# AlexGr5/StereoVision

Hardware: AMD Instinct MI355X
Metric: disparity frames/sec + HBM GB/s, 1920x1080 D=128 win=9, 1/2/4/8 GPU (higher is better)
Workload: dtype u8

## Files before the change

stereovision_amd/csrc/sv_capi.cpp:

```cpp
#include "sv_ctx.h"

namespace {
thread_local std::string g_err;
}

namespace svc {

int fail(int code, const std::string& msg) {
    g_err = msg;
    return code;
}

int hipfail(int e, const char* what) {
    return fail(SV_EHIP, std::string(what) + ": " + hipGetErrorString((hipError_t)e));
}

const std::string& last_error_msg() { return g_err; }

int check_image(const void* a, int H, int W) {
    if (!a || H <= 0 || W <= 0) return fail(SV_EINVAL, "null image or non-positive size");
    return 0;
}

int check_match(int H, int W, int min_disp, int num_disp, int win, int cost, sv::MatchPlan* plan) {
    if (H <= 0 || W <= 0) return fail(SV_EINVAL, "non-positive image size");
    if (num_disp <= 0 || num_disp > 512) return fail(SV_EINVAL, "num_disp must be in [1, 512]");
    if (win < 1 || win > 15 || (win & 1) == 0) return fail(SV_EINVAL, "win must be odd in [1, 15]");
    if (min_disp < -2047 || min_disp + num_disp - 1 > 2047)
        return fail(SV_EINVAL, "disparity range beyond the int16 x16 map: min_disp >= -2047 and "
                               "min_disp + num_disp - 1 <= 2047 required");
    if (cost == SV_COST_SGBM) return 0;
    int rc = sv::plan_match(num_disp, win, cost, plan);
    if (rc == -34) return fail(SV_ERANGE, "cost range too large for the argmin key");
    if (rc != 0) return fail(SV_EINVAL, "unsupported (num_disp, win, cost)");
    return 0;
}

SgbmParams sgbm_reference_params(int win) {
    return {8 * 3 * win * win, 32 * 3 * win * win, 1, 63, 10, 100, 32};
}

int enqueue_speckles(sv_ctx* c, int16_t* d_img, int H, int W, int pitch, int new_val, int max_speckle_size,
                     int max_diff, hipStream_t s, int nf, long long fimg) {
    if (max_speckle_size <= 0) return 0;
    c->scratch_written(d_img);
    const size_t n = (size_t)H * W * (nf < 1 ? 1 : nf);
    SV_HIP(c->cc_parent.ensure(n * 4));
    SV_HIP(c->cc_size.ensure(n * 4));
    SV_LAUNCH(c, SV_K_SPECKLE, s,
              sv::launch_speckles(d_img, H, W, pitch, new_val, max_speckle_size, max_diff, c->cc_parent.as<int>(),
                                  c->cc_size.as<int>(), s, nf < 1 ? 1 : nf, fimg));
    return 0;
}

constexpr int kSgbmChunk = 32;
size_t sgbm_budget(int device) {
    static const long long env_gb = [] {
        const char* e = std::getenv("SV_SGBM_BUDGET_GB");
        return e ? std::atoll(e) : 0LL;
    }();
    if (env_gb > 0) return (size_t)env_gb << 30;
    size_t fr = 0, tot = 0;
    (void)device;
    if (hipMemGetInfo(&fr, &tot) != hipSuccess || fr == 0) return (size_t)8 << 30;
    return std::min<size_t>(fr / 4, (size_t)48 << 30);
}

int enqueue_sgbm(sv_ctx* c, const uint8_t* L, const uint8_t* R, int H, int W, int pitch, int min_disp,
                 int num_disp, int win, SgbmParams p, int16_t* out, int opitch, hipStream_t s, int nf,
                 long long fs_in, long long fs_out) {
    if (nf < 1) nf = 1;
    c->scratch_written(out);
    if (sv::sgbm_dp(num_disp) < 0) return fail(SV_EINVAL, "num_disp must be in [1, 512]");
    if (W > 16384) return fail(SV_EINVAL, "SGBM: width beyond 16384");
    if (p.P1 < 0 || p.P2 < 0) return fail(SV_EINVAL, "negative P1/P2");
    if (p.P2 <= p.P1) p.P2 = p.P1 + 1;
    if (p.P2 >= 349525) return fail(SV_ERANGE, "SGBM: P2 too large for the 32-bit argmin key");
    p.cap = (p.cap > 15 ? p.cap : 15) | 1;
    if (p.cap > 127) return fail(SV_EINVAL, "preFilterCap must be <= 127");
    sv::SgbmArgs a{};
    a.L = L;
    a.R = R;
    a.H = H;
    a.W = W;
    a.pitch = pitch;
    a.minD = min_disp;
    a.D = num_disp;
    a.r = win / 2;
    const int maxd = min_disp + num_disp;
    a.X0 = maxd > 0 ? maxd : 0;
    int X1 = W + (min_disp < 0 ? min_disp : 0);
    if (X1 > W) X1 = W;
    a.Wb = X1 > a.X0 ? X1 - a.X0 : 0;
    a.cap = p.cap;
    a.P1 = p.P1;
    a.P2 = p.P2;
    a.uniq = p.uniq < 0 ? 10 : p.uniq;
    a.disp12 = p.disp12;
    const long long cmax = (long long)(2 * p.cap + 63) * win * win;
    if (cmax > 65535) return fail(SV_EINVAL, "SGBM: window cost beyond 16 bits (lower preFilterCap/blockSize)");
    a.l32 = (cmax > 32767 || p.P2 > 32768) ? 1 : 0;
    a.Dp = sv::sgbm_dp(num_disp);
    const size_t vol = (size_t)H * a.Wb * a.Dp;
    const size_t lsz = a.l32 ? 4 : 2;
    const bool cost1 = sv::sgbm_cost_fused(num_disp, a.r);
    const size_t rec_frame = cost1 ? (size_t)2 * H * W * 16 : 0;
    const size_t per_frame = vol * (4 + lsz * 3) + (size_t)H * a.Wb * 8 + rec_frame;
    const size_t held = c->sg_hsum.cap + c->sg_c.cap + c->sg_l.cap + c->sg_lt.cap + c->sg_band.cap + c->sg_rec.cap;
    const size_t kSgbmBudget = std::max(sgbm_budget(c->device) + held, per_frame);
    int chunk = (int)std::max<size_t>(1, std::min<size_t>({(size_t)nf, (size_t)kSgbmChunk,
                                                            kSgbmBudget / std::max<size_t>(per_frame, 1)}));
    const bool fused = sv::sgbm_fused(chunk, num_disp);
    if (fused)
        chunk = (int)std::max<size_t>(1, std::min<size_t>({(size_t)nf, (size_t)kSgbmChunk,
                                                            kSgbmBudget / (per_frame - vol * lsz)}));
    a.fused = fused ? 1 : 0;
    SV_HIP(c->sg_hsum.ensure(vol * 2 * chunk + 256));
    SV_HIP(c->sg_c.ensure(vol * 2 * chunk + 256));
    const int nl = (a.l32 ? 1 : 0) + (fused ? 0 : 1);
    SV_HIP(c->sg_l.ensure(vol * lsz * nl * chunk + 256));
    SV_HIP(c->sg_lt.ensure(vol * (a.l32 ? 4 : 2) * chunk + 256));
    if (!c->sg_aux) {
        SV_HIP(hipStreamCreateWithFlags(&c->sg_aux, hipStreamNonBlocking));
        SV_HIP(hipEventCreateWithFlags(&c->sg_ev[0], hipEventDisableTiming));
        SV_HIP(hipEventCreateWithFlags(&c->sg_ev[1], hipEventDisableTiming));
    }
    const size_t band_bytes = (size_t)H * a.Wb * 8 * chunk;
    SV_HIP(c->sg_band.ensure(band_bytes + 256 + 64 * 128));
    a.hsum = c->sg_hsum.as<uint16_t>();
    a.C = c->sg_c.as<uint16_t>();
    a.Llr = a.l32 ? c->sg_l.p : c->sg_hsum.p;
    a.Lrl = fused ? nullptr : a.l32 ? (void*)(c->sg_l.as<int32_t>() + vol * chunk) : c->sg_l.p;
    a.Ltb = c->sg_lt.p;
    a.band = c->sg_band.p;
    a.recs = nullptr;
    if (cost1) {
        SV_HIP(c->sg_rec.ensure(rec_frame * chunk + 256));
        a.recs = c->sg_rec.as<uint4>();
    }
    a.dummy = c->sg_band.as<uint8_t>() + (band_bytes + 255) / 256 * 256;
    a.opitch = opitch;
    a.fs_in = fs_in;
    a.fs_out = fs_out;
    for (int z0 = 0; z0 < nf; z0 += chunk) {
        const int n = std::min(chunk, nf - z0);
        a.L = L + z0 * fs_in;
        a.R = R + z0 * fs_in;
        a.out = out + z0 * fs_out;
        SV_LAUNCH(c, SV_K_SGBM, s, sv::launch_sgbm(a, n, s, c->sg_aux, c->sg_ev[0], c->sg_ev[1]));
        const int rc = enqueue_speckles(c, a.out, H, W, opitch, (min_disp - 1) * 16, p.speckle_win,
                                        16 * p.speckle_range, s, n, fs_out);
        if (rc) return rc;
    }
    return 0;
}

int enqueue_disparity(sv_ctx* c, const uint8_t* L, const uint8_t* R, int H, int W, int pitch,
                      int min_disp, int num_disp, int win, int cost, int row0, int row1,
                      int16_t* out, int opitch, hipStream_t s, int nf, long long fs_in,
                      long long fs_out, bool track_margins) {
    sv::MatchPlan plan;
    int rc = check_match(H, W, min_disp, num_disp, win, cost, &plan);
    if (rc) return rc;
    if (row0 < 0) row0 = 0;
    if (row1 > H) row1 = H;
    if (row1 <= row0) return 0;
    const sv_ctx::MarginKey had = c->d16_margins;
    c->scratch_written(out);
    if (cost == SV_COST_SGBM) {
        if (row0 != 0 || row1 != H) return fail(SV_EINVAL, "SGBM cannot compute a row band (use frames)");
        return enqueue_sgbm(c, L, R, H, W, pitch, min_disp, num_disp, win, sgbm_reference_params(win), out, opitch,
                            s, nf, fs_in, fs_out);
    }
    sv::MatchParams a{};
    a.L = L;
    a.R = R;
    a.H = H;
    a.W = W;
    a.pitch = pitch;
    a.minD = min_disp;
    a.D = num_disp;
    a.win = win;
    a.r = cost == SV_COST_HOG ? 0 : win / 2;
    int maxd = min_disp + num_disp;
    a.X0 = maxd > 0 ? maxd : 0;
    a.X1 = W + (min_disp < 0 ? min_disp : 0);
    if (a.X1 > W) a.X1 = W;
    if (a.X1 < a.X0) a.X1 = a.X0;
    a.row0 = row0;
    a.row1 = row1;
    a.lpg = plan.lpg;
    a.lpg_log2 = plan.lpg == 16 ? 4 : plan.lpg == 32 ? 5 : 6;
    a.dbits = plan.dbits;
    a.pad_key = (uint32_t)((sv::max_cost(win, cost) + 1) << plan.dbits);
    a.out = out;
    a.opitch = opitch;
    a.nf = nf < 1 ? 1 : nf;
    a.fs_in = fs_in;
    a.fs_out = fs_out;
    a.fs_hist = 0;
    if (cost == SV_COST_HOG && a.X1 > a.X0) {
        const long long fh = (long long)H * W * 10;
        const size_t hb = (size_t)fh * sizeof(uint16_t) * a.nf;
        SV_HIP(c->hog[0].ensure(hb));
        SV_HIP(c->hog[1].ensure(hb));
        SV_LAUNCH(c, SV_K_HOG, s,
                  sv::launch_hog_hist_pairs(L, R, H, W, pitch, win, row0, row1, c->hog[0].as<uint16_t>(),
                                            c->hog[1].as<uint16_t>(), a.nf, a.nf > 1 ? fs_in : 0, fh, s));
        a.HL = c->hog[0].as<uint16_t>();
        a.HR = c->hog[1].as<uint16_t>();
        a.fs_hist = a.nf > 1 ? fh : 0;
    }
    if (sv::ring_split(cost, win, num_disp) && a.X1 > a.X0) {
        const long long ke = sv::ring_split_elems(a.nf, fs_out, row1, opitch);
        SV_HIP(c->keys.ensure((size_t)(2 * ke) * sizeof(uint32_t)));
        a.keys = c->keys.as<uint32_t>();
        a.keys_stride = ke;
    }
    sv_ctx::MarginKey key;
    if (track_margins && out == c->d16.as<int16_t>() && row0 == 0 && row1 == H) {
        key.valid = true;
        key.p = c->d16.p;
        key.gen = c->d16.gen;
        key.H = H;
        key.W = W;
        key.opitch = opitch;
        key.X0 = a.X0;
        key.X1 = a.X1;
        key.min_disp = min_disp;
        key.nf = a.nf;
        key.fs_out = fs_out;
        a.margins_done = had.covers(key) ? 1 : 0;
        if (a.margins_done) key = had;
    }
    SV_LAUNCH(c, SV_K_MATCH, s, sv::launch_match(a, plan, cost, s));
    if (key.valid) c->d16_margins = key;
    return 0;
}

int attach_lut(sv_ctx* c, sv::PostParams& pp, hipStream_t s, bool whole) {
    pp.lut_n = 0;
    pp.lut_shift = 0;
    pp.lut_cap = 0;
    if (pp.mode == SV_POST_NONE || pp.num_disp <= 0 || pp.num_disp > 512) return 0;
    sv_ctx::LutKey k;
    k.mode = pp.mode;
    k.min_disp = pp.min_disp;
    k.num_disp = pp.num_disp;
    k.m0 = (pp.min_disp - 1) * 16;
    k.n = whole ? pp.num_disp + 1 : (pp.num_disp + 1) * 16;
    k.minf = pp.minf;
    k.maxf = pp.maxf;
    k.rangef = pp.rangef;
    k.mdg = pp.min_disp_global;
    DevBuf& buf = whole ? c->lutw : c->lut;
    sv_ctx::LutKey& key = whole ? c->lutw_key : c->lut_key;
    hipEvent_t& ev = whole ? c->lutw_ev : c->lut_ev;
    hipStream_t& bs = whole ? c->lutw_stream : c->lut_stream;
    const size_t n = (size_t)k.n;
    float* la = buf.as<float>();
    if (!(k == key) || !ev) {
        SV_HIP(buf.ensure(whole ? (n + sv::kLutWholeSpan) * 2 * sizeof(float) : n * (2 * sizeof(float) + 1)));
        la = buf.as<float>();
        if (!ev) SV_HIP(hipEventCreateWithFlags(&ev, hipEventDisableTiming));
        int e = sv::launch_post_lut(pp, k.m0, k.n, whole ? 16 : 1, la, reinterpret_cast<uint8_t*>(la + 2 * n), la + n,
                                    s);
        if (e) return hipfail(e, "launch_post_lut");
        SV_HIP(hipEventRecord(ev, s));
        key = k;
        bs = s;
    } else if (s != bs) {
        SV_HIP(hipStreamWaitEvent(s, ev, 0));
    }
    pp.lut_a = la;
    pp.lut_b = la + n;
    pp.lut_u8 = reinterpret_cast<const uint8_t*>(la + 2 * n);
    pp.lut_m0 = k.m0;
    pp.lut_n = k.n;
    pp.lut_shift = whole ? 4 : 0;
    pp.lut_cap = whole ? k.n + sv::kLutWholeSpan : k.n;
    return 0;
}

int attach_cmap(sv_ctx* c, sv::PostParams& pp, const uint8_t* table, uint8_t* d_bgr, hipStream_t s) {
    pp.out_bgr = nullptr;
    pp.cmap = nullptr;
    if (!d_bgr) return 0;
    if (!table) return fail(SV_EINVAL, "colormap output without a table");
    SV_HIP(c->cmap.ensure(256 * sizeof(uint32_t)));
    if (!c->cmap_valid || std::memcmp(c->cmap_host, table, 768) != 0) {
        uint32_t packed[256];
        for (int i = 0; i < 256; ++i)
            packed[i] = (uint32_t)table[3 * i] | ((uint32_t)table[3 * i + 1] << 8) | ((uint32_t)table[3 * i + 2] << 16);
        SV_HIP(hipMemcpyAsync(c->cmap.p, packed, sizeof(packed), hipMemcpyHostToDevice, s));
        SV_HIP(hipStreamSynchronize(s));
        std::memcpy(c->cmap_host, table, 768);
        c->cmap_valid = true;
    }
    pp.out_bgr = d_bgr;
    pp.cmap = c->cmap.as<uint32_t>();
    return 0;
}

sv::PostParams make_post(int mode, float minf, float maxf, float rangef, float mdg, int min_disp,
                         int num_disp, float* a, uint8_t* u8, float* b) {
    sv::PostParams pp{};
    pp.mode = mode;
    pp.minf = minf;
    pp.maxf = maxf;
    pp.rangef = rangef;
    pp.min_disp_global = mdg;
    pp.min_disp = min_disp;
    pp.num_disp = num_disp;
    pp.out_a = a;
    pp.out_u8 = u8;
    pp.out_b = b;
    return pp;
}

int map_out_post(sv_ctx* c, const sv_map_out* out, int min_disp, int num_disp, int cost, bool allow_harris,
                 hipStream_t s, sv::PostParams* pp, float** disp) {
    if (!out) return fail(SV_EINVAL, "null outputs");
    const int mode = out->mode;
    if (mode != SV_POST_NONE && mode != SV_POST_DEPTH && mode != SV_POST_SCALED) return fail(SV_EINVAL, "bad post mode");
    if (mode == SV_POST_DEPTH && (!out->out_a || !out->out_u8)) return fail(SV_EINVAL, "depth post outputs missing");
    if (mode == SV_POST_SCALED && (!out->out_a || !out->out_u8 || !out->out_b || num_disp <= 0))
        return fail(SV_EINVAL, "scaled post outputs missing");
    if (mode == SV_POST_NONE && (out->out_a || out->out_u8 || out->out_b))
        return fail(SV_EINVAL, "post outputs without a post mode");
    if (out->bgr && (mode == SV_POST_NONE || !out->cmap_bgr))
        return fail(SV_EINVAL, "a colormap output needs a post mode and a table");
    if (out->harris && !allow_harris) return fail(SV_EINVAL, "the Harris output belongs to sv_depth_map_batch_dev");
    if (out->d8 && (cost == SV_COST_SGBM || num_disp < 1 || num_disp > 255))
        return fail(SV_EINVAL, "u8 disparity indices need an integer-disparity cost and num_disp <= 255");
    if (!out->disparity && !out->med16 && !out->d8 && mode == SV_POST_NONE && !out->harris)
        return fail(SV_EINVAL, "no outputs");
    *pp = make_post(mode, out->min_depth, out->max_depth, out->depth_range, out->min_disp_global, min_disp, num_disp,
                    out->out_a, out->out_u8, out->out_b);
    int rc = attach_lut(c, *pp, s, cost != SV_COST_SGBM);
    if (!rc) rc = attach_cmap(c, *pp, out->cmap_bgr, out->bgr, s);
    if (rc) return rc;
    pp->out_m16 = out->med16;
    pp->out_d8 = out->d8;
    pp->d8_base = min_disp - 1;
    *disp = out->disparity;
    return 0;
}

int check_map(int fmt, const void* map, int cost, int num_disp) {
    if (fmt != SV_MAP_M16 && fmt != SV_MAP_D8) return fail(SV_EINVAL, "map format must be SV_MAP_M16 or SV_MAP_D8");
    if (!map) return fail(SV_EINVAL, "null map");
    if (fmt == SV_MAP_D8 && (cost == SV_COST_SGBM || num_disp < 1 || num_disp > 255))
        return fail(SV_EINVAL, "u8 disparity indices need an integer-disparity cost and num_disp <= 255");
    return 0;
}

sv::PostParams map_post(int fmt, void* dst, int d8_base) {
    sv::PostParams pp = make_post(SV_POST_NONE, 0.f, 0.f, 0.f, 0.f, 0, 0, nullptr, nullptr, nullptr);
    if (fmt == SV_MAP_D8) {
        pp.out_d8 = static_cast<uint8_t*>(dst);
        pp.d8_base = d8_base;
    } else {
        pp.out_m16 = static_cast<int16_t*>(dst);
    }
    return pp;
}


int stage_pair(sv_ctx* c, const uint8_t* left, const uint8_t* right, int H, int W, int channels,
               int stride) {
    if (check_image(left, H, W) || check_image(right, H, W)) return SV_EINVAL;
    if (channels != 1 && channels != 3) return fail(SV_EINVAL, "channels must be 1 or 3");
    const size_t row = (size_t)W * channels;
    if (stride < (int)row) return fail(SV_EINVAL, "stride smaller than a row");
    const size_t n = row * H;
    SV_HIP(c->hin.ensure(2 * n));
    SV_HIP(c->gray[0].ensure((size_t)H * W));
    SV_HIP(c->gray[1].ensure((size_t)H * W));
    const uint8_t* src[2] = {left, right};
    for (int k = 0; k < 2; ++k) {
        uint8_t* dst = c->hin.as<uint8_t>() + k * n;
        if ((size_t)stride == row) {
            std::memcpy(dst, src[k], n);
        } else {
            for (int y = 0; y < H; ++y) std::memcpy(dst + y * row, src[k] + (size_t)y * stride, row);
        }
    }
    if (channels == 1) {
        SV_HIP(hipMemcpyAsync(c->gray[0].p, c->hin.p, n, hipMemcpyHostToDevice, c->stream));
        SV_HIP(hipMemcpyAsync(c->gray[1].p, c->hin.as<uint8_t>() + n, n, hipMemcpyHostToDevice, c->stream));
    } else {
        SV_HIP(c->img[0].ensure(n));
        SV_HIP(c->img[1].ensure(n));
        for (int k = 0; k < 2; ++k) {
            SV_HIP(hipMemcpyAsync(c->img[k].p, c->hin.as<uint8_t>() + k * n, n, hipMemcpyHostToDevice, c->stream));
            SV_LAUNCH(c, SV_K_GRAY, c->stream,
                      sv::launch_gray(c->img[k].as<uint8_t>(), H, W, (int)row, c->gray[k].as<uint8_t>(), c->stream));
        }
    }
    return 0;
}

int collect(sv_ctx* c, const Out* outs, int n) {
    size_t total = 0;
    for (int i = 0; i < n; ++i)
        if (outs[i].host) total += (outs[i].bytes + 255) & ~(size_t)255;
    SV_HIP(c->hout.ensure(total ? total : 256));
    size_t off = 0;
    for (int i = 0; i < n; ++i) {
        if (!outs[i].host) continue;
        SV_HIP(hipMemcpyAsync(c->hout.as<uint8_t>() + off, outs[i].dev, outs[i].bytes, hipMemcpyDeviceToHost, c->stream));
        off += (outs[i].bytes + 255) & ~(size_t)255;
    }
    SV_HIP(hipStreamSynchronize(c->stream));
    off = 0;
    for (int i = 0; i < n; ++i) {
        if (!outs[i].host) continue;
        std::memcpy(outs[i].host, c->hout.as<uint8_t>() + off, outs[i].bytes);
        off += (outs[i].bytes + 255) & ~(size_t)255;
    }
    return 0;
}

int make_undistort(const double* K, const double* dist, int ndist, const double* R, const double* P,
                   int p_cols, int H, int W, sv::UndistortParams* out) {
    if (!K || H <= 0 || W <= 0) return fail(SV_EINVAL, "bad map arguments");
    if (H > 32767 || W > 32767) return fail(SV_EINVAL, "map size beyond the int16 coordinate range");
    if (!(ndist == 0 || ndist == 4 || ndist == 5 || ndist == 8 || ndist == 12 || ndist == 14) ||
        (ndist > 0 && !dist))
        return fail(SV_EINVAL, "distCoeffs must have 0, 4, 5, 8, 12 or 14 elements");
    if (ndist == 14 && (dist[12] != 0.0 || dist[13] != 0.0))
        return fail(SV_EINVAL, "tilted sensor model (tauX, tauY != 0) is not supported");
    if (P && p_cols != 3 && p_cols != 4) return fail(SV_EINVAL, "P must be 3x3 or 3x4");
    double A[9], Rm[9] = {1, 0, 0, 0, 1, 0, 0, 0, 1}, M[9];
    for (int i = 0; i < 3; ++i)
        for (int j = 0; j < 3; ++j) A[i * 3 + j] = P ? P[i * p_cols + j] : K[i * 3 + j];
    if (R) std::memcpy(Rm, R, sizeof(Rm));
    for (int i = 0; i < 3; ++i)
        for (int j = 0; j < 3; ++j)
            M[i * 3 + j] = (A[i * 3 + 0] * Rm[0 * 3 + j] + A[i * 3 + 1] * Rm[1 * 3 + j]) + A[i * 3 + 2] * Rm[2 * 3 + j];
    auto a = [&](int i, int j) { return M[i * 3 + j]; };
    const double det = a(0, 0) * (a(1, 1) * a(2, 2) - a(2, 1) * a(1, 2)) -
                       a(0, 1) * (a(1, 0) * a(2, 2) - a(2, 0) * a(1, 2)) +
                       a(0, 2) * (a(1, 0) * a(2, 1) - a(2, 0) * a(1, 1));
    if (det == 0.0) return fail(SV_EINVAL, "singular newCameraMatrix * R");
    const double d = 1.0 / det;
    double* b = out->ir;
    b[0] = (a(1, 1) * a(2, 2) - a(1, 2) * a(2, 1)) * d;
    b[1] = (a(0, 2) * a(2, 1) - a(0, 1) * a(2, 2)) * d;
    b[2] = (a(0, 1) * a(1, 2) - a(0, 2) * a(1, 1)) * d;
    b[3] = (a(1, 2) * a(2, 0) - a(1, 0) * a(2, 2)) * d;
    b[4] = (a(0, 0) * a(2, 2) - a(0, 2) * a(2, 0)) * d;
    b[5] = (a(0, 2) * a(1, 0) - a(0, 0) * a(1, 2)) * d;
    b[6] = (a(1, 0) * a(2, 1) - a(1, 1) * a(2, 0)) * d;
    b[7] = (a(0, 1) * a(2, 0) - a(0, 0) * a(2, 1)) * d;
    b[8] = (a(0, 0) * a(1, 1) - a(0, 1) * a(1, 0)) * d;
    out->fx = K[0];
    out->fy = K[4];
    out->u0 = K[2];
    out->v0 = K[5];
    for (int i = 0; i < 12; ++i) out->k[i] = i < ndist ? dist[i] : 0.0;
    out->H = H;
    out->W = W;
    return 0;
}

int check_remap(const void* src, int sH, int sW, int channels, int pitch, const void* map1, int H, int W,
                const void* dst) {
    if (!src || !map1 || !dst || sH <= 0 || sW <= 0 || H <= 0 || W <= 0)
        return fail(SV_EINVAL, "bad remap arguments");
    if (channels != 1 && channels != 3) return fail(SV_EINVAL, "channels must be 1 or 3");
    if (pitch < sW * channels) return fail(SV_EINVAL, "source pitch smaller than a row");
    return 0;
}

}

int sv::set_error(int code, const std::string& msg) { return fail(code, msg); }

extern "C" {

int sv_version(void) { return SV_API_VERSION; }

const char* sv_last_error(void) { return g_err.c_str(); }

int sv_device_count(int* n) {
    if (!n) return fail(SV_EINVAL, "null output");
    int k = 0;
    hipError_t e = hipGetDeviceCount(&k);
    if (e != hipSuccess) {
        *n = 0;
        return hipfail((int)e, "hipGetDeviceCount");
    }
    *n = k;
    return 0;
}

int sv_create(int device, sv_ctx** out) {
    if (!out) return fail(SV_EINVAL, "null output");
    *out = nullptr;
    int n = 0;
    if (hipGetDeviceCount(&n) != hipSuccess || n <= 0) return fail(SV_ENODEV, "no HIP device visible");
    if (device < 0 || device >= n) return fail(SV_ENODEV, "device index out of range");
    sv_ctx* c = new (std::nothrow) sv_ctx();
    if (!c) return fail(SV_ENOMEM, "context allocation failed");
    c->device = device;
    hipError_t e = hipSetDevice(device);
    if (e == hipSuccess) e = hipStreamCreateWithFlags(&c->stream, hipStreamNonBlocking);
    if (e != hipSuccess) {
        delete c;
        return hipfail((int)e, "sv_create");
    }
    *out = c;
    return 0;
}

void sv_destroy(sv_ctx* c) {
    if (!c) return;
    {
        std::lock_guard<std::mutex> lk(c->mu);
        (void)hipSetDevice(c->device);
        (void)hipStreamSynchronize(c->stream);
        c->prof_drain();
        for (auto e : c->pool) (void)hipEventDestroy(e);
        DevBuf* bufs[] = {&c->img[0], &c->img[1], &c->gray[0], &c->gray[1], &c->d16, &c->fa, &c->fb,
                          &c->fc, &c->u8, &c->harris, &c->hog[0], &c->hog[1], &c->fin, &c->lut,
                          &c->rmap1, &c->rmap2, &c->rdst[0], &c->rdst[1], &c->stats, &c->sel,
                          &c->sg_hsum, &c->sg_c, &c->sg_l, &c->sg_lt, &c->sg_band, &c->cc_parent,
                          &c->hist_copies, &c->cmap, &c->bgr, &c->m16,
                          &c->cc_size, &c->sg_rec, &c->gm16, &c->keys, &c->lutw, &c->fuse, &c->flow};
        if (c->lut_ev) (void)hipEventDestroy(c->lut_ev);
        if (c->lutw_ev) (void)hipEventDestroy(c->lutw_ev);
        if (c->scr_ev) (void)hipEventDestroy(c->scr_ev);
        if (c->xev) (void)hipEventDestroy(c->xev);
        if (c->sev) (void)hipEventDestroy(c->sev);
        if (c->gev) (void)hipEventDestroy(c->gev);
        for (auto e : c->wev)
            if (e) (void)hipEventDestroy(e);
        if (c->region_open) {
            (void)hipEventDestroy(c->region.a);
            (void)hipEventDestroy(c->region.b);
        }
        for (auto e : c->dev_done)
            if (e) (void)hipEventDestroy(e);
        for (auto e : c->tmr)
            if (e) (void)hipEventDestroy(e);
        if (c->sg_aux) {
            (void)hipStreamSynchronize(c->sg_aux);
            (void)hipStreamDestroy(c->sg_aux);
        }
        for (auto e : c->sg_ev)
            if (e) (void)hipEventDestroy(e);
        for (auto* b : bufs) b->release();
        c->hin.release();
        c->hout.release();
        (void)hipStreamDestroy(c->stream);
    }
    delete c;
}

int sv_event_record(sv_ctx* c, int slot, void* stream) {
    SV_ENTER(c);
    if (slot < 0 || slot >= 16) return fail(SV_EINVAL, "event slot must be in [0, 16)");
    hipEvent_t& e = c->wev[slot];
    if (!e) SV_HIP(hipEventCreateWithFlags(&e, hipEventDisableTiming));
    SV_HIP(hipEventRecord(e, pick(c, stream)));
    return 0;
}

int sv_stream_wait_event(sv_ctx* c, int slot, void* stream) {
    SV_ENTER(c);
    if (slot < 0 || slot >= 16 || !c->wev[slot]) return fail(SV_EINVAL, "event slot never recorded");
    SV_HIP(hipStreamWaitEvent(pick(c, stream), c->wev[slot], 0));
    return 0;
}

int sv_release_scratch(sv_ctx* c) {
    SV_ENTER(c);
    SV_HIP(hipStreamSynchronize(c->stream));
    if (c->sg_aux) SV_HIP(hipStreamSynchronize(c->sg_aux));
    DevBuf* bufs[] = {&c->img[0], &c->img[1], &c->gray[0], &c->gray[1], &c->d16, &c->fa, &c->fb, &c->fc,
                      &c->u8, &c->harris, &c->hog[0], &c->hog[1], &c->fin, &c->sg_hsum, &c->sg_c,
                      &c->sg_l, &c->sg_lt, &c->sg_band, &c->sg_rec, &c->cc_parent, &c->cc_size, &c->m16,
                      &c->gm16, &c->keys, &c->flow};
    for (auto* b : bufs) b->release();
    c->d16_margins.valid = false;
    return 0;
}

int sv_synchronize(sv_ctx* c) {
    SV_ENTER(c);
    SV_HIP(hipStreamSynchronize(c->stream));
    return 0;
}

void* sv_stream(sv_ctx* c) { return c ? static_cast<void*>(c->stream) : nullptr; }

int sv_plan(int num_disp, int win, int cost, int* dpl, int* lpg, int* lds_bytes) {
    sv::MatchPlan p;
    int rc = sv::plan_match(num_disp, win, cost, &p);
    if (rc == -34) return fail(SV_ERANGE, "cost range too large for the argmin key");
    if (rc) return fail(SV_EINVAL, "unsupported (num_disp, win, cost)");
    if (dpl) *dpl = p.dpl;
    if (lpg) *lpg = p.lpg;
    if (lds_bytes) *lds_bytes = (int)sv::match_lds_bytes(p, cost == SV_COST_HOG ? 0 : win / 2, cost);
    return 0;
}

int sv_dev_alloc(sv_ctx* c, uint64_t bytes, void** out) {
    SV_ENTER(c);
    if (!out || bytes == 0) return fail(SV_EINVAL, "bad allocation request");
    *out = nullptr;
    SV_HIP(hipMalloc(out, (size_t)bytes));
    return 0;
}

int sv_dev_free(sv_ctx* c, void* p) {
    SV_ENTER(c);
    if (p) SV_HIP(hipFree(p));
    return 0;
}

int sv_copy_to_device(sv_ctx* c, void* dst, const void* src, uint64_t bytes, void* stream) {
    SV_ENTER(c);
    if (!dst || !src) return fail(SV_EINVAL, "null pointer");
    if (!bytes) return 0;
    if (stream) {
        SV_HIP(hipMemcpyAsync(dst, src, (size_t)bytes, hipMemcpyHostToDevice, static_cast<hipStream_t>(stream)));
        return 0;
    }
    SV_HIP(hipMemcpyAsync(dst, src, (size_t)bytes, hipMemcpyHostToDevice, c->stream));
    SV_HIP(hipStreamSynchronize(c->stream));
    return 0;
}

int sv_copy_to_host(sv_ctx* c, void* dst, const void* src, uint64_t bytes, void* stream) {
    SV_ENTER(c);
    if (!dst || !src) return fail(SV_EINVAL, "null pointer");
    if (!bytes) return 0;
    if (stream) {
        SV_HIP(hipMemcpyAsync(dst, src, (size_t)bytes, hipMemcpyDeviceToHost, static_cast<hipStream_t>(stream)));
        return 0;
    }
    SV_HIP(hipStreamSynchronize(c->stream));
    SV_HIP(hipMemcpyAsync(dst, src, (size_t)bytes, hipMemcpyDeviceToHost, c->stream));
    SV_HIP(hipStreamSynchronize(c->stream));
    return 0;
}

int sv_profile_enable(sv_ctx* c, int on) {
    SV_ENTER(c);
    c->prof = on != 0;
    while (c->prof && c->pool.size() + 2 * c->pending.size() < 1024) {
        hipEvent_t e = nullptr;
        if (hipEventCreate(&e) != hipSuccess) break;
        c->pool.push_back(e);
    }
    return 0;
}

int sv_profile_read(sv_ctx* c, int kernel, double* total_ms, long long* count) {
    SV_ENTER(c);
    if (kernel < 0 || kernel >= SV_NKERNELS) return fail(SV_EINVAL, "kernel id out of range");
    c->prof_drain();
    if (total_ms) *total_ms = c->acc_ms[kernel];
    if (count) *count = c->cnt[kernel];
    return 0;
}

int sv_timer_begin(sv_ctx* c, void* stream) {
    SV_ENTER(c);
    for (auto& e : c->tmr)
        if (!e) SV_HIP(hipEventCreate(&e));
    SV_HIP(hipEventRecord(c->tmr[0], pick(c, stream)));
    return 0;
}

int sv_timer_end(sv_ctx* c, void* stream, double* ms) {
    SV_ENTER(c);
    if (!c->tmr[0] || !ms) return fail(SV_EINVAL, "sv_timer_end without sv_timer_begin");
    SV_HIP(hipEventRecord(c->tmr[1], pick(c, stream)));
    SV_HIP(hipEventSynchronize(c->tmr[1]));
    float f = 0.f;
    SV_HIP(hipEventElapsedTime(&f, c->tmr[0], c->tmr[1]));
    *ms = f;
    return 0;
}

int sv_profile_region_begin(sv_ctx* c, int kernel, void* stream) {
    SV_ENTER(c);
    if (kernel < 0 || kernel >= SV_NKERNELS) return fail(SV_EINVAL, "kernel id out of range");
    if (c->region_open) return fail(SV_EINVAL, "profiling regions do not nest");
    if (!c->prof) return 0;
    c->region.a = c->get_event();
    c->region.b = c->get_event();
    c->region.kid = kernel;
    SV_HIP(hipEventRecord(c->region.a, pick(c, stream)));
    c->region_open = true;
    return 0;
}

int sv_profile_region_end(sv_ctx* c, void* stream) {
    SV_ENTER(c);
    if (!c->region_open) return 0;
    c->region_open = false;
    SV_HIP(hipEventRecord(c->region.b, pick(c, stream)));
    c->pending.push_back(c->region);
    return 0;
}

int sv_profile_reset(sv_ctx* c) {
    SV_ENTER(c);
    c->prof_drain();
    for (int k = 0; k < SV_NKERNELS; ++k) {
        c->acc_ms[k] = 0.0;
        c->cnt[k] = 0;
    }
    return 0;
}

}
```

stereovision_amd/csrc/sv_capi_dev.cpp:

```cpp
#include "sv_ctx.h"

extern "C" {

int sv_gray_dev(sv_ctx* c, const uint8_t* d_bgr, int H, int W, int pitch, uint8_t* d_gray, void* stream) {
    SV_ENTER(c);
    if (check_image(d_bgr, H, W) || !d_gray) return fail(SV_EINVAL, "bad gray arguments");
    hipStream_t s = pick(c, stream);
    SV_LAUNCH(c, SV_K_GRAY, s, sv::launch_gray(d_bgr, H, W, pitch, d_gray, s));
    return 0;
}

int sv_disparity_dev(sv_ctx* c, const uint8_t* d_left, const uint8_t* d_right, int H, int W, int pitch,
                     int min_disp, int num_disp, int win, int cost, int row0, int row1, int16_t* d_disp16,
                     int out_pitch, void* stream) {
    SV_ENTER(c);
    if (check_image(d_left, H, W) || check_image(d_right, H, W) || !d_disp16)
        return fail(SV_EINVAL, "bad disparity arguments");
    if (pitch < W || out_pitch < W) return fail(SV_EINVAL, "pitch smaller than width");
    hipStream_t s = pick(c, stream);
    SV_SCRATCH(c, s);
    return enqueue_disparity(c, d_left, d_right, H, W, pitch, min_disp, num_disp, win, cost, row0, row1,
                             d_disp16, out_pitch, s);
}

int sv_median_rows_dev(sv_ctx* c, const int16_t* d_disp16, int H, int W, int row0, int row1, int min_disp,
                       int num_disp, int cost, const sv_map_out* out, void* stream) {
    SV_ENTER(c);
    if (check_image(d_disp16, H, W)) return fail(SV_EINVAL, "bad median arguments");
    if ((long long)H * W >= (1LL << 30)) return fail(SV_EINVAL, "frame too large for the median kernel");
    if (row0 < 0) row0 = 0;
    if (row1 > H) row1 = H;
    hipStream_t s = pick(c, stream);
    SV_SCRATCH(c, s);
    sv::PostParams pp;
    float* disp = nullptr;
    int rc = map_out_post(c, out, min_disp, num_disp, cost, false, s, &pp, &disp);
    if (rc) return rc;
    SV_LAUNCH(c, SV_K_MEDIAN, s, sv::launch_median_i16(d_disp16, H, W, row0, row1, disp, pp, s));
    return 0;
}

int sv_post_m16_dev(sv_ctx* c, const int16_t* d_med16, int64_t n, int mode, float min_depth, float max_depth,
                    float depth_range, float min_disp_global, int min_disp, int num_disp, float* d_disparity,
                    float* d_out_a, uint8_t* d_out_u8, float* d_out_b, void* stream) {
    SV_ENTER(c);
    if (n < 0 || (n > 0 && !d_med16)) return fail(SV_EINVAL, "bad median map");
    if (mode != SV_POST_NONE && mode != SV_POST_DEPTH && mode != SV_POST_SCALED) return fail(SV_EINVAL, "bad mode");
    if (mode == SV_POST_NONE && !d_disparity) return fail(SV_EINVAL, "no outputs");
    if (mode == SV_POST_DEPTH && (!d_out_a || !d_out_u8)) return fail(SV_EINVAL, "depth post outputs missing");
    if (mode == SV_POST_SCALED && (!d_out_a || !d_out_u8 || !d_out_b || num_disp <= 0))
        return fail(SV_EINVAL, "scaled post outputs missing");
    if (n == 0) return 0;
    hipStream_t s = pick(c, stream);
    SV_SCRATCH(c, s);
    sv::PostParams pp = make_post(mode, min_depth, max_depth, depth_range, min_disp_global, min_disp, num_disp,
                                  d_out_a, d_out_u8, d_out_b);
    int rc = attach_lut(c, pp, s);
    if (rc) return rc;
    SV_LAUNCH(c, SV_K_POST, s, sv::launch_post_m16(d_med16, (long long)n, d_disparity, pp, s));
    return 0;
}

int sv_disparity_batch_dev(sv_ctx* c, const uint8_t* d_left, const uint8_t* d_right, int n_frames, int H,
                           int W, int pitch, int64_t frame_stride, int min_disp, int num_disp, int win,
                           int cost, int16_t* d_disp16, int out_pitch, int64_t out_frame_stride,
                           void* stream) {
    SV_ENTER(c);
    if (check_image(d_left, H, W) || check_image(d_right, H, W) || !d_disp16 || n_frames < 0)
        return fail(SV_EINVAL, "bad disparity arguments");
    if (pitch < W || out_pitch < W) return fail(SV_EINVAL, "pitch smaller than width");
    if (n_frames > 1 && (frame_stride < (int64_t)pitch * H || out_frame_stride < (int64_t)out_pitch * H))
        return fail(SV_EINVAL, "frame stride smaller than a frame");
    if (n_frames == 0) return 0;
    hipStream_t s = pick(c, stream);
    SV_SCRATCH(c, s);
    return enqueue_disparity(c, d_left, d_right, H, W, pitch, min_disp, num_disp, win, cost, 0, H, d_disp16,
                             out_pitch, s, n_frames, frame_stride, out_frame_stride);
}

int sv_depth_map_batch_dev(sv_ctx* c, const uint8_t* d_left, const uint8_t* d_right, int n_frames, int H, int W,
                           int pitch, int64_t frame_stride, int min_disp, int num_disp, int win, int cost, int stages,
                           int16_t* d_disp16, const sv_map_out* out, void* stream) {
    SV_ENTER(c);
    if (stages != SV_STAGE_ALL && stages != SV_STAGE_MATCH && stages != SV_STAGE_MEDIAN)
        return fail(SV_EINVAL, "stages must be SV_STAGE_MATCH, SV_STAGE_MEDIAN or SV_STAGE_ALL");
    const bool match = stages & SV_STAGE_MATCH, median = stages & SV_STAGE_MEDIAN;
    if (n_frames < 0 || H <= 0 || W <= 0) return fail(SV_EINVAL, "bad depth-map arguments");
    if (match && (check_image(d_left, H, W) || check_image(d_right, H, W)))
        return fail(SV_EINVAL, "bad depth-map arguments");
    if (!d_disp16 && stages != SV_STAGE_ALL)
        return fail(SV_EINVAL, "the stages run apart exchange the int16 maps through d_disp16");
    if (median && !out) return fail(SV_EINVAL, "null outputs");
    if (median && out->harris && check_image(d_left, H, W)) return fail(SV_EINVAL, "Harris needs the left frames");
    if (pitch < W) return fail(SV_EINVAL, "pitch smaller than width");
    if (n_frames > 1 && frame_stride < (int64_t)pitch * H) return fail(SV_EINVAL, "frame stride smaller than a frame");
    if ((long long)H * W >= (1LL << 30)) return fail(SV_EINVAL, "frame too large for the median kernel");
    if (n_frames == 0) return 0;
    hipStream_t s = pick(c, stream);
    SV_SCRATCH(c, s);
    const long long fs = (long long)H * W;
    int16_t* d16 = d_disp16;
    if (!d16) {
        SV_HIP(c->d16.ensure((size_t)n_frames * fs * sizeof(int16_t)));
        d16 = c->d16.as<int16_t>();
    }
    if (match) {
        const int rc = enqueue_disparity(c, d_left, d_right, H, W, pitch, min_disp, num_disp, win, cost, 0, H, d16, W,
                                         s, n_frames, frame_stride, fs, !d_disp16);
        if (rc) return rc;
    }
    if (!median) return 0;
    sv::PostParams pp;
    float* disp = nullptr;
    int rc = map_out_post(c, out, min_disp, num_disp, cost, true, s, &pp, &disp);
    if (rc) return rc;
    pp.lut_unchecked = match && cost != SV_COST_SGBM && pp.lut_shift == 4 && pp.lut_m0 == (min_disp - 1) * 16 &&
                       pp.lut_n == num_disp + 1;
    const long long fin = n_frames > 1 ? frame_stride : 0;
    if (out->harris && (W < 8 || H < 8)) {
        SV_LAUNCH(c, SV_K_MEDIAN, s, sv::launch_median_i16(d16, H, W, 0, H, disp, pp, s, n_frames, fs, fs));
        SV_LAUNCH(c, SV_K_HARRIS, s, sv::launch_harris(d_left, H, W, pitch, out->harris, s, n_frames, fin, fs));
        return 0;
    }
    sv::HarrisParams hp{d_left, pitch, fin, out->harris, fs, 0, 0};
    SV_LAUNCH(c, SV_K_MEDIAN, s,
              sv::launch_median_i16(d16, H, W, 0, H, disp, pp, s, n_frames, fs, fs, out->harris ? &hp : nullptr));
    return 0;
}

int sv_harris_dev(sv_ctx* c, const uint8_t* d_gray, int H, int W, int pitch, float* d_out, void* stream) {
    SV_ENTER(c);
    if (check_image(d_gray, H, W) || !d_out) return fail(SV_EINVAL, "bad harris arguments");
    hipStream_t s = pick(c, stream);
    SV_LAUNCH(c, SV_K_HARRIS, s, sv::launch_harris(d_gray, H, W, pitch, d_out, s));
    return 0;
}

int sv_harris_batch_dev(sv_ctx* c, const uint8_t* d_gray, int n_frames, int H, int W, int pitch,
                        int64_t frame_stride, float* d_out, void* stream) {
    SV_ENTER(c);
    if (check_image(d_gray, H, W) || !d_out || n_frames < 0) return fail(SV_EINVAL, "bad harris arguments");
    if (pitch < W) return fail(SV_EINVAL, "pitch smaller than width");
    if (n_frames > 1 && frame_stride < (int64_t)pitch * H) return fail(SV_EINVAL, "frame stride smaller than a frame");
    if (n_frames == 0) return 0;
    hipStream_t s = pick(c, stream);
    SV_LAUNCH(c, SV_K_HARRIS, s,
              sv::launch_harris(d_gray, H, W, pitch, d_out, s, n_frames, (long long)frame_stride,
                                (long long)H * W));
    return 0;
}

int sv_hog_hist_dev(sv_ctx* c, const uint8_t* d_gray, int H, int W, int pitch, int win, int row0, int row1,
                    uint16_t* d_out, void* stream) {
    SV_ENTER(c);
    if (check_image(d_gray, H, W) || !d_out) return fail(SV_EINVAL, "bad hog arguments");
    if (win < 1 || win > 15 || (win & 1) == 0) return fail(SV_EINVAL, "win must be odd in [1, 15]");
    hipStream_t s = pick(c, stream);
    SV_LAUNCH(c, SV_K_HOG, s, sv::launch_hog_hist(d_gray, H, W, pitch, win, row0, row1, d_out, s));
    return 0;
}

int sv_gray(sv_ctx* c, const uint8_t* bgr, int H, int W, int stride, uint8_t* gray) {
    SV_ENTER(c);
    SV_SCRATCH(c, c->stream);
    if (check_image(bgr, H, W) || !gray) return fail(SV_EINVAL, "bad gray arguments");
    const size_t row = (size_t)W * 3, n = row * H;
    if (stride < (int)row) return fail(SV_EINVAL, "stride smaller than a row");
    SV_HIP(c->hin.ensure(n));
    for (int y = 0; y < H; ++y) std::memcpy(c->hin.as<uint8_t>() + y * row, bgr + (size_t)y * stride, row);
    SV_HIP(c->img[0].ensure(n));
    SV_HIP(c->gray[0].ensure((size_t)H * W));
    SV_HIP(hipMemcpyAsync(c->img[0].p, c->hin.p, n, hipMemcpyHostToDevice, c->stream));
    SV_LAUNCH(c, SV_K_GRAY, c->stream,
              sv::launch_gray(c->img[0].as<uint8_t>(), H, W, (int)row, c->gray[0].as<uint8_t>(), c->stream));
    Out o[] = {{gray, c->gray[0].p, (size_t)H * W}};
    return collect(c, o, 1);
}

int sv_disparity(sv_ctx* c, const uint8_t* left, const uint8_t* right, int H, int W, int channels, int stride,
                 int min_disp, int num_disp, int win, int cost, int16_t* disp16, float* harris) {
    SV_ENTER(c);
    SV_SCRATCH(c, c->stream);
    if (!disp16) return fail(SV_EINVAL, "null disparity output");
    sv::MatchPlan plan;
    int rc = check_match(H, W, min_disp, num_disp, win, cost, &plan);
    if (rc) return rc;
    rc = stage_pair(c, left, right, H, W, channels, stride);
    if (rc) return rc;
    SV_HIP(c->d16.ensure((size_t)H * W * sizeof(int16_t)));
    rc = enqueue_disparity(c, c->gray[0].as<uint8_t>(), c->gray[1].as<uint8_t>(), H, W, W, min_disp, num_disp,
                           win, cost, 0, H, c->d16.as<int16_t>(), W, c->stream);
    if (rc) return rc;
    if (harris) {
        SV_HIP(c->harris.ensure((size_t)H * W * sizeof(float)));
        SV_LAUNCH(c, SV_K_HARRIS, c->stream,
                  sv::launch_harris(c->gray[0].as<uint8_t>(), H, W, W, c->harris.as<float>(), c->stream));
    }
    Out o[] = {{disp16, c->d16.p, (size_t)H * W * sizeof(int16_t)},
               {harris, c->harris.p, (size_t)H * W * sizeof(float)}};
    return collect(c, o, 2);
}

int sv_disparity_rows(sv_ctx* c, const uint8_t* left, const uint8_t* right, int H, int W, int channels,
                      int stride, int min_disp, int num_disp, int win, int cost, int row0, int row1,
                      int16_t* disp16) {
    SV_ENTER(c);
    SV_SCRATCH(c, c->stream);
    if (!disp16) return fail(SV_EINVAL, "null disparity output");
    if (row0 < 0) row0 = 0;
    if (row1 > H) row1 = H;
    if (row1 <= row0) return 0;
    sv::MatchPlan plan;
    int rc = check_match(H, W, min_disp, num_disp, win, cost, &plan);
    if (rc) return rc;
    rc = stage_pair(c, left, right, H, W, channels, stride);
    if (rc) return rc;
    SV_HIP(c->d16.ensure((size_t)H * W * sizeof(int16_t)));
    rc = enqueue_disparity(c, c->gray[0].as<uint8_t>(), c->gray[1].as<uint8_t>(), H, W, W, min_disp, num_disp,
                           win, cost, row0, row1, c->d16.as<int16_t>(), W, c->stream);
    if (rc) return rc;
    const size_t off = (size_t)row0 * W;
    Out o[] = {{disp16 + off, c->d16.as<int16_t>() + off, (size_t)(row1 - row0) * W * sizeof(int16_t)}};
    return collect(c, o, 1);
}


int sv_median5_f32(sv_ctx* c, const float* in, int H, int W, float* out) {
    SV_ENTER(c);
    SV_SCRATCH(c, c->stream);
    if (check_image(in, H, W) || !out) return fail(SV_EINVAL, "bad median arguments");
    const size_t n = (size_t)H * W * sizeof(float);
    SV_HIP(c->hin.ensure(n));
    SV_HIP(c->fin.ensure(n));
    SV_HIP(c->fa.ensure(n));
    std::memcpy(c->hin.p, in, n);
    SV_HIP(hipMemcpyAsync(c->fin.p, c->hin.p, n, hipMemcpyHostToDevice, c->stream));
    SV_LAUNCH(c, SV_K_MEDIAN, c->stream, sv::launch_median_f32(c->fin.as<float>(), H, W, c->fa.as<float>(), c->stream));
    Out o[] = {{out, c->fa.p, n}};
    return collect(c, o, 1);
}

static int post_common(sv_ctx* c, const float* disparity, int n, const sv::PostParams& tmpl, float* a,
                       uint8_t* u8, float* b) {
    if (!disparity || n <= 0) return fail(SV_EINVAL, "bad post arguments");
    const size_t nb = (size_t)n * sizeof(float);
    SV_HIP(c->hin.ensure(nb));
    SV_HIP(c->fin.ensure(nb));
    SV_HIP(c->fa.ensure(nb));
    SV_HIP(c->fb.ensure(nb));
    SV_HIP(c->u8.ensure((size_t)n));
    std::memcpy(c->hin.p, disparity, nb);
    SV_HIP(hipMemcpyAsync(c->fin.p, c->hin.p, nb, hipMemcpyHostToDevice, c->stream));
    sv::PostParams pp = tmpl;
    pp.out_a = c->fa.as<float>();
    pp.out_u8 = c->u8.as<uint8_t>();
    pp.out_b = c->fb.as<float>();
    SV_LAUNCH(c, SV_K_POST, c->stream, sv::launch_post(c->fin.as<float>(), n, pp, c->stream));
    Out o[] = {{a, c->fa.p, nb}, {u8, c->u8.p, (size_t)n}, {b, c->fb.p, nb}};
    return collect(c, o, 3);
}

int sv_depth_post(sv_ctx* c, const float* disparity, int n, float min_depth, float max_depth, float depth_range,
                  float min_disp_global, float* depth_final, uint8_t* depth_normalized) {
    SV_ENTER(c);
    SV_SCRATCH(c, c->stream);
    if (!depth_final || !depth_normalized) return fail(SV_EINVAL, "null outputs");
    sv::PostParams pp = make_post(SV_POST_DEPTH, min_depth, max_depth, depth_range, min_disp_global, 0, 0,
                                  nullptr, nullptr, nullptr);
    return post_common(c, disparity, n, pp, depth_final, depth_normalized, nullptr);
}

int sv_scaled_post(sv_ctx* c, const float* disparity, int n, int min_disp, int num_disp,
                   float* disparity_normalized, uint8_t* normalized_u8, float* confidence) {
    SV_ENTER(c);
    SV_SCRATCH(c, c->stream);
    if (!disparity_normalized || !normalized_u8 || !confidence || num_disp <= 0)
        return fail(SV_EINVAL, "bad scaled post arguments");
    sv::PostParams pp = make_post(SV_POST_SCALED, 0.f, 0.f, 0.f, 0.f, min_disp, num_disp, nullptr, nullptr,
                                  nullptr);
    return post_common(c, disparity, n, pp, disparity_normalized, normalized_u8, confidence);
}

}

namespace {

std::mutex g_reg_mu;
std::map<uintptr_t, size_t> g_reg;

bool host_registered(const void* p, size_t bytes) {
    if (!p) return false;
    const uintptr_t a = reinterpret_cast<uintptr_t>(p);
    std::lock_guard<std::mutex> lk(g_reg_mu);
    auto it = g_reg.upper_bound(a);
    if (it == g_reg.begin()) return false;
    --it;
    return a >= it->first && a + bytes <= it->first + it->second;
}

int stage_rows(sv_ctx* c, const uint8_t* src, int y0, int y1, size_t row, int stride, uint8_t* stage, uint8_t* dev,
               int nsub) {
    if ((size_t)stride == row) {
        SV_HIP(hipMemcpyAsync(dev + (size_t)y0 * row, src + (size_t)y0 * row, (size_t)(y1 - y0) * row,
                              hipMemcpyHostToDevice, c->stream));
        return 0;
    }
    sv::HostPool& pool = sv::HostPool::get();
    for (int k = 0; k < nsub; ++k) {
        const int a0 = y0 + (int)((long long)(y1 - y0) * k / nsub), a1 = y0 + (int)((long long)(y1 - y0) * (k + 1) / nsub);
        if (a1 <= a0) continue;
        const int parts = pool.threads();
        pool.parallel_for(parts, [&](int p) {
            const int a = a0 + (int)((long long)(a1 - a0) * p / parts), b = a0 + (int)((long long)(a1 - a0) * (p + 1) / parts);
            if (b <= a) return;
            if ((size_t)stride == row)
                std::memcpy(stage + (size_t)a * row, src + (size_t)a * row, (size_t)(b - a) * row);
            else
                for (int y = a; y < b; ++y) std::memcpy(stage + (size_t)y * row, src + (size_t)y * stride, row);
        });
        SV_HIP(hipMemcpyAsync(dev + (size_t)a0 * row, stage + (size_t)a0 * row, (size_t)(a1 - a0) * row,
                              hipMemcpyHostToDevice, c->stream));
    }
    return 0;
}

int host_lut(sv_ctx* c, const sv::PostParams& pp) {
    if (c->hl_valid && c->hl_key == c->lut_key) return 0;
    const size_t n = (size_t)pp.lut_n;
    try {
        c->hl_a.resize(n);
        c->hl_b.resize(n);
        c->hl_u8.resize(n);
    } catch (...) {
        return fail(SV_ENOMEM, "host table allocation failed");
    }
    SV_HIP(hipMemcpyAsync(c->hl_a.data(), pp.lut_a, n * sizeof(float), hipMemcpyDeviceToHost, c->stream));
    SV_HIP(hipMemcpyAsync(c->hl_b.data(), pp.lut_b, n * sizeof(float), hipMemcpyDeviceToHost, c->stream));
    SV_HIP(hipMemcpyAsync(c->hl_u8.data(), pp.lut_u8, n, hipMemcpyDeviceToHost, c->stream));
    SV_HIP(hipStreamSynchronize(c->stream));
    c->hl_key = c->lut_key;
    c->hl_valid = true;
    return 0;
}

struct FrameOut {
    float* a;
    float* disp;
    uint8_t* u8;
    float* b;
    uint8_t* bgr;
};

template <bool U8, bool SCALED, bool BGR>
int expand_rows(const int16_t* med, size_t a, size_t b, int m0, int nl, const HostEnt* ent, const float* lb,
                const FrameOut& o) {
    for (size_t i = a; i < b; ++i) o.disp[i] = (float)med[i] * 0.0625f;
    int nbad = 0;
    for (size_t i = a; i < b; ++i) {
        const uint32_t li = (uint32_t)(med[i] - m0);
        if (__builtin_expect(li >= (uint32_t)nl, 0)) {
            ++nbad;
            continue;
        }
        const HostEnt e = ent[li];
        o.a[i] = e.a;
        if (U8) o.u8[i] = (uint8_t)e.ubgr;
        if (SCALED) o.b[i] = lb[li];
        if (BGR) {
            const uint32_t v = e.ubgr >> 8;
            uint8_t* d = o.bgr + 3 * i;
            if (i + 1 < b) std::memcpy(d, &v, 4);
            else std::memcpy(d, &v, 3);
        }
    }
    return nbad;
}

struct HostProf {
    std::atomic<bool> on{std::getenv("SV_HOST_PROFILE") != nullptr};
    bool print = std::getenv("SV_HOST_PROFILE") != nullptr;
    std::mutex mu;
    double t[6] = {0, 0, 0, 0, 0, 0};
    double acc[6] = {0, 0, 0, 0, 0, 0};
    long n = 0, nacc = 0;
    void add(const double* d) {
        std::lock_guard<std::mutex> lk(mu);
        for (int i = 0; i < 6; ++i) {
            t[i] += d[i];
            acc[i] += d[i];
        }
        ++nacc;
        if (print && ++n % 200 == 0) {
            std::fprintf(stderr, "[sv host] per call (ms): prepare %.3f  stage+issue %.3f  wait-first %.3f  expand %.3f  "
                         "wait-rest %.3f  total %.3f\n", t[0] / n, t[1] / n, t[2] / n, t[3] / n, t[4] / n, t[5] / n);
            for (double& v : t) v = 0;
            n = 0;
        }
    }
};
HostProf& host_prof() {
    static HostProf* p = new HostProf();
    return *p;
}
int env_int(const char* name, int dflt, int lo, int hi) {
    const char* e = std::getenv(name);
    if (!e) return dflt;
    const int v = std::atoi(e);
    return v < lo ? lo : v > hi ? hi : v;
}
double now_ms() {
    return std::chrono::duration<double, std::milli>(std::chrono::steady_clock::now().time_since_epoch()).count();
}

int host_frame_path(sv_ctx* c, const uint8_t* left, const uint8_t* right, int H, int W, int channels, int stride,
                    int min_disp, int num_disp, int win, int cost, sv::PostParams pp, const uint8_t* table,
                    FrameOut o) {
    const bool prof = host_prof().on;
    double tm[6] = {0, 0, 0, 0, 0, 0}, t0 = prof ? now_ms() : 0, tp = t0;
    sv::MatchPlan plan;
    int rc = check_match(H, W, min_disp, num_disp, win, cost, &plan);
    if (rc) return rc;
    if ((long long)H * W >= (1LL << 30)) return fail(SV_EINVAL, "frame too large");
    if (check_image(left, H, W) || check_image(right, H, W)) return SV_EINVAL;
    if (channels != 1 && channels != 3) return fail(SV_EINVAL, "channels must be 1 or 3");
    const size_t row = (size_t)W * channels;
    if (stride < (int)row) return fail(SV_EINVAL, "stride smaller than a row");
    const size_t n = (size_t)H * W;
    SV_HIP(c->hin.ensure(2 * row * H));
    SV_HIP(c->gray[0].ensure(n));
// ... 1036 lines not shown
```

stereovision_amd/csrc/sv_ctx.h:

```cpp
#pragma once
#include <cstdio>
#include <cstdlib>
#include <algorithm>
#include <chrono>
#include <cstring>
#include <map>
#include <mutex>
#include <thread>
#include <new>
#include <string>
#include <vector>

#include "sv_internal.h"
#include "sv_pool.h"
#include "../../include/stereovision_amd.h"

namespace svc {
int fail(int code, const std::string& msg);
int hipfail(int e, const char* what);
const std::string& last_error_msg();
}
using svc::fail;
using svc::hipfail;

#define SV_HIP(call)                                               \
    do {                                                           \
        hipError_t e_ = (call);                                    \
        if (e_ != hipSuccess) return hipfail((int)e_, #call);      \
    } while (0)

#define SV_LAUNCH(ctx, kid, stream, call)                          \
    do {                                                           \
        (ctx)->prof_begin((kid), (stream));                        \
        int e_ = (call);                                           \
        if (e_ != 0) {                                             \
            (ctx)->prof_abort();                                   \
            return hipfail(e_, #call);                             \
        }                                                          \
        (ctx)->prof_end((stream));                                 \
    } while (0)

struct DevBuf {
    void* p = nullptr;
    size_t cap = 0;
    unsigned long long gen = 0;
    hipError_t ensure(size_t n) {
        if (n <= cap) return hipSuccess;
        ++gen;
        if (p) (void)hipFree(p);
        p = nullptr;
        cap = 0;
        hipError_t e = hipMalloc(&p, n);
        if (e == hipSuccess) cap = n;
        return e;
    }
    void release() {
        ++gen;
        if (p) (void)hipFree(p);
        p = nullptr;
        cap = 0;
    }
    hipError_t ensure_zeroed(size_t n) {
        if (n <= cap) return hipSuccess;
        hipError_t e = ensure(n);
        if (e == hipSuccess) e = hipMemset(p, 0, cap);
        if (e == hipSuccess) e = hipDeviceSynchronize();
        return e;
    }
    template <class T> T* as() const { return static_cast<T*>(p); }
};

struct HostBuf {
    void* p = nullptr;
    size_t cap = 0;
    hipError_t ensure(size_t n) {
        if (n <= cap) return hipSuccess;
        if (p) (void)hipHostFree(p);
        p = nullptr;
        cap = 0;
        hipError_t e = hipHostMalloc(&p, n, hipHostMallocDefault);
        if (e == hipSuccess) cap = n;
        return e;
    }
    void release() {
        if (p) (void)hipHostFree(p);
        p = nullptr;
        cap = 0;
    }
    template <class T> T* as() const { return static_cast<T*>(p); }
};

struct EvPair {
    hipEvent_t a, b;
    int kid;
};

struct HostEnt {
    float a;
    uint32_t ubgr;
};

struct sv_ctx {
    int device = 0;
    hipStream_t stream = nullptr;
    std::mutex mu;
    DevBuf img[2], gray[2], d16, fa, fb, fc, u8, harris, hog[2], fin, lut, rmap1, rmap2, rdst[2], stats, sel,
        sg_hsum, sg_c, sg_l, sg_lt, sg_band, sg_rec, cc_parent, cc_size, hist_copies, cmap, bgr;
    DevBuf fuse;
    DevBuf flow;
    uint8_t cmap_host[768] = {};
    bool cmap_valid = false;
    DevBuf m16;
    DevBuf gm16;
    DevBuf keys;
    std::vector<float> hl_a, hl_b;
    std::vector<uint8_t> hl_u8;
    std::vector<HostEnt> hl_ent;
    bool hl_valid = false;
    hipEvent_t dev_done[8] = {};
    hipEvent_t tmr[2] = {nullptr, nullptr};
    hipStream_t sg_aux = nullptr;
    hipEvent_t sg_ev[2] = {nullptr, nullptr};
    struct LutKey {
        int mode = -1, min_disp = 0, num_disp = 0, m0 = 0, n = 0;
        float minf = 0, maxf = 0, rangef = 0, mdg = 0;
        bool operator==(const LutKey& o) const {
            return mode == o.mode && min_disp == o.min_disp && num_disp == o.num_disp && m0 == o.m0 &&
                   n == o.n && std::memcmp(&minf, &o.minf, sizeof(float)) == 0 &&
                   std::memcmp(&maxf, &o.maxf, sizeof(float)) == 0 &&
                   std::memcmp(&rangef, &o.rangef, sizeof(float)) == 0 &&
                   std::memcmp(&mdg, &o.mdg, sizeof(float)) == 0;
        }
    } lut_key, hl_key;
    hipEvent_t lut_ev = nullptr;
    hipStream_t lut_stream = nullptr;
    DevBuf lutw;
    LutKey lutw_key;
    hipEvent_t lutw_ev = nullptr;
    hipStream_t lutw_stream = nullptr;
    HostBuf hin, hout;
    struct MarginKey {
        bool valid = false;
        const void* p = nullptr;
        unsigned long long gen = 0;
        int H = 0, W = 0, opitch = 0, X0 = 0, X1 = 0, min_disp = 0, nf = 0;
        long long fs_out = 0;
        bool covers(const MarginKey& o) const {
            return valid && p == o.p && gen == o.gen && H == o.H && W == o.W && opitch == o.opitch &&
                   X0 == o.X0 && X1 == o.X1 && min_disp == o.min_disp && nf >= o.nf &&
                   (o.nf <= 1 || fs_out == o.fs_out);
        }
    } d16_margins;
    void scratch_written(const void* out) {
        const char* b = static_cast<const char*>(d16.p);
        const char* o = static_cast<const char*>(out);
        if (b && o >= b && o < b + d16.cap) d16_margins.valid = false;
    }
    hipStream_t scr_stream = nullptr;
    hipEvent_t scr_ev = nullptr;
    hipEvent_t xev = nullptr;
    hipEvent_t sev = nullptr;
    hipEvent_t gev = nullptr;
    hipEvent_t wev[16] = {};
    bool prof = false;
    std::vector<EvPair> pending;
    std::vector<hipEvent_t> pool;
    double acc_ms[SV_NKERNELS] = {};
    long long cnt[SV_NKERNELS] = {};
    EvPair cur{};
    bool cur_open = false;
    EvPair region{};
    bool region_open = false;

    hipEvent_t get_event() {
        if (!pool.empty()) {
            hipEvent_t e = pool.back();
            pool.pop_back();
            return e;
        }
        hipEvent_t e = nullptr;
        (void)hipEventCreate(&e);
        return e;
    }
    void prof_begin(int kid, hipStream_t s) {
        if (!prof) return;
        cur.a = get_event();
        cur.b = get_event();
        cur.kid = kid;
        cur_open = true;
        (void)hipEventRecord(cur.a, s);
    }
    void prof_end(hipStream_t s) {
        if (!prof || !cur_open) return;
        (void)hipEventRecord(cur.b, s);
        pending.push_back(cur);
        cur_open = false;
    }
    void prof_abort() {
        if (!cur_open) return;
        pool.push_back(cur.a);
        pool.push_back(cur.b);
        cur_open = false;
    }
    void prof_drain() {
        for (auto& p : pending) {
            (void)hipEventSynchronize(p.b);
            float ms = 0.f;
            if (hipEventElapsedTime(&ms, p.a, p.b) == hipSuccess) {
                acc_ms[p.kid] += ms;
                cnt[p.kid] += 1;
            }
            pool.push_back(p.a);
            pool.push_back(p.b);
        }
        pending.clear();
    }
};

inline hipStream_t pick(sv_ctx* c, void* s) { return s ? static_cast<hipStream_t>(s) : c->stream; }

struct ProfScope {
    sv_ctx* c;
    hipStream_t s;
    bool ok = false;
    ProfScope(sv_ctx* ctx, int kid, hipStream_t stream) : c(ctx), s(stream) { c->prof_begin(kid, s); }
    void done() { ok = true; }
    ~ProfScope() {
        if (ok) c->prof_end(s);
        else c->prof_abort();
    }
};

namespace svc {

struct SgbmParams {
    int P1, P2, disp12, cap, uniq, speckle_win, speckle_range;
};
SgbmParams sgbm_reference_params(int win);

int check_image(const void* a, int H, int W);
int check_match(int H, int W, int min_disp, int num_disp, int win, int cost, sv::MatchPlan* plan);
int enqueue_speckles(sv_ctx* c, int16_t* d_img, int H, int W, int pitch, int new_val, int max_speckle_size,
                     int max_diff, hipStream_t s, int nf = 1, long long fimg = 0);
int enqueue_sgbm(sv_ctx* c, const uint8_t* L, const uint8_t* R, int H, int W, int pitch, int min_disp,
                 int num_disp, int win, SgbmParams p, int16_t* out, int opitch, hipStream_t s, int nf = 1,
                 long long fs_in = 0, long long fs_out = 0);
int enqueue_disparity(sv_ctx* c, const uint8_t* L, const uint8_t* R, int H, int W, int pitch,
                      int min_disp, int num_disp, int win, int cost, int row0, int row1,
                      int16_t* out, int opitch, hipStream_t s, int nf = 1, long long fs_in = 0,
                      long long fs_out = 0, bool track_margins = false);
int attach_lut(sv_ctx* c, sv::PostParams& pp, hipStream_t s, bool whole = false);
int attach_cmap(sv_ctx* c, sv::PostParams& pp, const uint8_t* table, uint8_t* d_bgr, hipStream_t s);
sv::PostParams make_post(int mode, float minf, float maxf, float rangef, float mdg, int min_disp,
                         int num_disp, float* a, uint8_t* u8, float* b);

int map_out_post(sv_ctx* c, const sv_map_out* out, int min_disp, int num_disp, int cost, bool allow_harris,
                 hipStream_t s, sv::PostParams* pp, float** disp);

struct MapOut {
    int fmt = 0;
    void* map = nullptr;
    int d8_base = 0;
    size_t el() const { return fmt == SV_MAP_D8 ? 1 : 2; }
};
int check_map(int fmt, const void* map, int cost, int num_disp);
sv::PostParams map_post(int fmt, void* dst, int d8_base);

int stage_pair(sv_ctx* c, const uint8_t* left, const uint8_t* right, int H, int W, int channels, int stride);

struct Out {
    void* host;
    const void* dev;
    size_t bytes;
};
int collect(sv_ctx* c, const Out* outs, int n);

int make_undistort(const double* K, const double* dist, int ndist, const double* R, const double* P,
                   int p_cols, int H, int W, sv::UndistortParams* out);
int check_remap(const void* src, int sH, int sW, int channels, int pitch, const void* map1, int H, int W,
                const void* dst);

}
using namespace svc;

struct ScratchUse {
    sv_ctx* c;
    hipStream_t s;
    int rc = 0;
    ScratchUse(sv_ctx* ctx, hipStream_t stream) : c(ctx), s(stream) {
        if (c->scr_stream && c->scr_stream != s && c->scr_ev) {
            hipError_t e = hipStreamWaitEvent(s, c->scr_ev, 0);
            if (e != hipSuccess) rc = hipfail((int)e, "hipStreamWaitEvent (context scratch)");
        }
    }
    ~ScratchUse() {
        if (!c->scr_ev && hipEventCreateWithFlags(&c->scr_ev, hipEventDisableTiming) != hipSuccess) {
            c->scr_ev = nullptr;
            return;
        }
        if (hipEventRecord(c->scr_ev, s) == hipSuccess) c->scr_stream = s;
    }
};

#define SV_SCRATCH(ctx, stream)                                             \
    ScratchUse scratch_(ctx, stream);                                       \
    if (scratch_.rc) return scratch_.rc

struct Guard {
    sv_ctx* c;
    std::unique_lock<std::mutex> lk;
    int rc = 0;
    explicit Guard(sv_ctx* ctx) : c(ctx), lk(ctx->mu) {
        hipError_t e = hipSetDevice(ctx->device);
        if (e != hipSuccess) rc = hipfail((int)e, "hipSetDevice");
    }
};

#define SV_ENTER(ctx)                                                       \
    if (!(ctx)) return fail(SV_EINVAL, "null context");                     \
    Guard guard_(ctx);                                                      \
    if (guard_.rc) return guard_.rc
```

stereovision_amd/csrc/sv_internal.h:

```cpp
#pragma once
#include <hip/hip_runtime.h>
#include <stdint.h>

#include <cstdlib>
#include <string>

struct sv_comm;

namespace sv {

__device__ __forceinline__ void sad_u32_acc(uint32_t& a, uint32_t b, uint32_t c) {
    asm("v_sad_u32 %0, %0, %1, %2" : "+v"(a) : "v"(b), "v"(c));
}

__device__ __forceinline__ int clampi(int v, int lo, int hi) { return min(max(v, lo), hi); }

__device__ __forceinline__ int bgr_to_gray(int b, int g, int r) {
    return (b * 1868 + g * 9617 + r * 4899 + (1 << 13)) >> 14;
}

inline bool env_flag(const char* name, bool default_on) {
    const char* e = std::getenv(name);
    return default_on ? !(e && e[0] == '0') : (e && e[0] == '1');
}
inline int env_int(const char* name, int lo, int hi) {
    const char* e = std::getenv(name);
    const int v = e ? std::atoi(e) : 0;
    return v >= lo && v <= hi ? v : 0;
}

int set_error(int code, const std::string& msg);

int comm_group_start();
int comm_group_end();
int comm_send(sv_comm* c, const void* buf, size_t bytes, int peer, hipStream_t s);
int comm_recv(sv_comm* c, void* buf, size_t bytes, int peer, hipStream_t s);
int comm_rank(const sv_comm* c);
int comm_size(const sv_comm* c);
int comm_device(const sv_comm* c);

enum Cost { COST_SAD = 0, COST_SSD = 1, COST_HOG = 2, COST_SGBM = 3 };

struct MatchPlan {
    int dpl;
    int lpg;
    int ndw;
    int dbits;
    int mfma_only = 0;
};

struct MatchParams {
    const uint8_t* L;
    const uint8_t* R;
    const uint16_t* HL;
    const uint16_t* HR;
    int H, W, pitch;
    int minD, D, r;
    int win;
    int X0, X1;
    int row0, row1;
    int lpg, lpg_log2, dbits;
    int16_t* out;
    int opitch;
    int nf;
    long long fs_in, fs_out, fs_hist;
    uint32_t pad_key;
    int segm;
    alignas(16) int xcd_map;
    uint32_t* keys;
    long long keys_stride;
    int margins_done;
};

int plan_match(int num_disp, int win, int cost, MatchPlan* plan);
uint64_t max_cost(int win, int cost);
size_t match_lds_bytes(const MatchPlan& p, int r, int cost);
int launch_match(const MatchParams& a, const MatchPlan& p, int cost, hipStream_t s);
bool ring_split(int cost, int win, int num_disp);
bool ring_ssd(int cost, int win, int num_disp);
bool ssd_mfma(int cost, int win, int num_disp);
bool ssd_mfma_fits(const MatchParams& a, int cost);
int launch_ssd_mfma(const MatchParams& a, hipStream_t s);
long long ring_split_elems(int nf, long long fs_out, int row1, int opitch);
int launch_fill_i16(int16_t* out, int opitch, int H, int W, int16_t v, hipStream_t s);

int launch_gray(const uint8_t* bgr, int H, int W, int pitch, uint8_t* gray, hipStream_t s);
int launch_harris(const uint8_t* g, int H, int W, int pitch, float* out, hipStream_t s, int nf = 1,
                  long long fs_in = 0, long long fs_out = 0);
int launch_hog_hist(const uint8_t* g, int H, int W, int pitch, int win, int row0, int row1,
                    uint16_t* hist, hipStream_t s);
int launch_hog_hist_pairs(const uint8_t* g0, const uint8_t* g1, int H, int W, int pitch, int win, int row0,
                          int row1, uint16_t* h0, uint16_t* h1, int nf, long long fs_in, long long fs_hist,
                          hipStream_t s);

struct UndistortParams {
    double ir[9];
    double fx, fy, u0, v0;
    double k[12];
    int H, W;
};
int launch_undistort_map(const UndistortParams& p, short2* map1, uint16_t* map2, hipStream_t s);
int launch_remap(const uint8_t* src, int sH, int sW, int channels, int spitch, long long sfs,
                 const short2* map1, const uint16_t* map2, int H, int W, bool gray_out, uint8_t* dst,
                 int dpitch, long long dfs, int nf, hipStream_t s);

int launch_resize_linear(const void* src, int sH, int sW, int cn, int spitch, long long sfs, void* dst,
                         int dH, int dW, int dpitch, long long dfs, int nf, bool f32, hipStream_t s);

struct FrameStatsArgs {
    const uint8_t* img0;
    const uint8_t* img1;
    int H, W, pitch, cn;
    int bh, bw;
    uint32_t* block_sum;
    uint32_t* block_sq;
    uint32_t* hist;
    uint32_t* hist_copies;
    int per;
    long long fs;
};
constexpr int kHistCopies = 8;
int launch_frame_stats(const FrameStatsArgs& a, int nimg, hipStream_t s);

enum SelectMask { SEL_ALL = 0, SEL_POSITIVE = 1, SEL_MASK_GT = 2 };
constexpr int kMaxRanks = 4;
constexpr int kSelBatch = 16;
struct SelectArgs {
    const float* x;
    const float* mask;
    float thr;
    int mask_mode;
    size_t n;
    int shift, bits;
    int nranks;
    int narr;
    size_t xstride, mstride;
    uint32_t prefix[kSelBatch][kMaxRanks];
    uint32_t* ghist;
    unsigned long long* counts;
    uint32_t* hist_out;
    unsigned long long* counts_out;
};
constexpr int kCountSlots = 32;
int launch_select_hist(const SelectArgs& a, hipStream_t s);

enum AffineMode { AFF_F32 = 0, AFF_F64 = 1, AFF_FILL = 2 };
struct AffineArgs {
    const float* x;
    float* out;
    size_t n;
    int mode;
    float fa, fb, fc, fd;
    double ds, doff;
};
int launch_affine_f32(const AffineArgs& a, hipStream_t s);

struct GaussArgs {
    const float* src;
    float* dst;
    int H, W, r;
    float c[16];
};
enum FuseBase { FUSE_BASE_STEREO = 0, FUSE_BASE_MIDAS = 1, FUSE_BASE_FLOW = 2 };
struct FuseBlendArgs {
    const float* stereo;
    const float* conf;
    const float* midas;
    const float* flow;
    float* fused;
    uint32_t* stats;
    int H, W, base;
    int midas_fill, flow_fill;
    int r;
    float sw, mfw, thr, hthr, k1, k2;
    float c[16];
};
constexpr int kBilateralMaxR = 7;
constexpr int kBilateralMaxTaps = 148;
constexpr int kBilateralLut = 4096 + 2;
struct BilateralArgs {
    const float* src;
    const float* lut;
    float* dst_f32;
    uint8_t* dst_u8;
    uint8_t* dst_bgr;
    const uint32_t* cmap;
    uint32_t* stats;
    int H, W, r, ntaps;
    float scale;
    float sw[kBilateralMaxTaps];
    short off[kBilateralMaxTaps];
};
int bilateral_taps(int r, int* dy, int* dx);
int launch_gauss_f32(const GaussArgs& a, hipStream_t s);
int launch_fuse_blend(const FuseBlendArgs& a, hipStream_t s);
int launch_bilateral_f32(BilateralArgs a, const float* space_w, hipStream_t s);
constexpr int kFuseSlots = 32, kFuseSlotStride = 32;
constexpr size_t kFuseStatsBytes = (size_t)kFuseSlots * kFuseSlotStride * sizeof(uint32_t);
inline void fuse_stats_fold(const uint32_t* slots, uint32_t w[4]) {
    w[0] = w[1] = w[2] = w[3] = 0;
    for (int s = 0; s < kFuseSlots; ++s) {
        const uint32_t* p = slots + s * kFuseSlotStride;
        w[0] = p[0] > w[0] ? p[0] : w[0];
        w[1] = p[1] > w[1] ? p[1] : w[1];
        w[2] += p[2];
        w[3] += p[3];
    }
}
inline float fuse_stat_decode(uint32_t k) {
    const uint32_t u = (k & 0x80000000u) ? (k ^ 0x80000000u) : ~k;
    float f;
    __builtin_memcpy(&f, &u, sizeof f);
    return f;
}
inline float fuse_stat_min(const uint32_t* w) { return fuse_stat_decode(~w[0]); }
inline float fuse_stat_max(const uint32_t* w) { return fuse_stat_decode(w[1]); }

constexpr int kFbMaxPolyN = 7;
constexpr int kFbMaxWin = 31;
struct FbPolyArgs {
    const float* src;
    float* R;
    size_t plane;
    int H, W, n;
    float g[kFbMaxPolyN + 1], xg[kFbMaxPolyN + 1], xxg[kFbMaxPolyN + 1];
    double ig11, ig03, ig33, ig55;
};
struct FbUpdateArgs {
    const float* R0;
    const float* R1;
    const float* flow;
    float* M;
    size_t plane;
    int H, W;
};
struct FbSolveArgs {
    const float* M;
    size_t plane;
    float* flow;
    int interleaved;
    int H, W, m;
    double scale;
};
struct FlowDepthArgs {
    const float* flow;
    float* depth;
    float* stable;
    uint32_t* stats;
    int H, W;
    double m[9];
    float alpha, beta;
};
int launch_fb_u8_f32(const uint8_t* src, int H, int W, int pitch, float* dst, hipStream_t s);
int launch_fb_scale(float* x, size_t n, float k, hipStream_t s);
int launch_fb_polyexp(const FbPolyArgs& a, hipStream_t s);
int launch_fb_update_matrices(const FbUpdateArgs& a, hipStream_t s);
int launch_fb_blur_solve(const FbSolveArgs& a, hipStream_t s);
int launch_flow_depth(const FlowDepthArgs& a, hipStream_t s);

struct SgbmArgs {
    const uint8_t* L;
    const uint8_t* R;
    int H, W, pitch;
    int minD, D, r;
    int Dp;
    int X0, Wb;
    int cap, P1, P2, uniq, disp12;
    uint16_t* hsum;
    uint16_t* C;
    void* Llr;
    void* Lrl;
    void* Ltb;
    int l32;
    int fused;
    uint4* recs;
    void* band;
    int16_t* out;
    int opitch;
    void* dummy;
    long long fs_in, fs_out;
    __device__ __forceinline__ void select_frame(int z) {
        const size_t vol = (size_t)H * Wb * Dp * z;
        L += z * fs_in;
        R += z * fs_in;
        out += z * fs_out;
        hsum += vol;
        C += vol;
        const size_t lb = vol * (l32 ? 4 : 2);
        Llr = static_cast<char*>(Llr) + lb;
        Lrl = static_cast<char*>(Lrl) + lb;
        Ltb = static_cast<char*>(Ltb) + lb;
        band = static_cast<char*>(band) + (size_t)H * Wb * 8 * z;
        if (recs) recs += (size_t)2 * H * W * z;
    }
};
int sgbm_dp(int D);
bool sgbm_fused(int nf, int D);
bool sgbm_cost_fused(int D, int r);
int launch_sgbm(const SgbmArgs& a, int nf, hipStream_t s, hipStream_t aux, hipEvent_t fork, hipEvent_t join);
int launch_speckles(int16_t* img, int H, int W, int pitch, int newv, int maxsize, int maxdiff, int* parent,
                    int* size, hipStream_t s, int nf = 1, long long fimg = 0);

enum PostMode { POST_NONE = 0, POST_DEPTH = 1, POST_SCALED = 2 };
struct PostParams {
    int mode;
    float minf, maxf, rangef, min_disp_global;
    int min_disp, num_disp;
    float* out_a;
    uint8_t* out_u8;
    float* out_b;
    uint8_t* out_bgr;
    const uint32_t* cmap;
    int16_t* out_m16;
    uint8_t* out_d8;
    int d8_base;
    const float* lut_a;
    const uint8_t* lut_u8;
    const float* lut_b;
    int lut_m0, lut_n;
    int lut_shift;
    int lut_unchecked;
    int lut_cap;
};
constexpr int kLutWholeSpan = 4096;
struct HarrisParams {
    const uint8_t* g;
    int pitch;
    long long fs_in;
    float* out;
    long long fs_out;
    int mbx;
    int form;
};
int launch_median_i16(const int16_t* in, int H, int W, int row0, int row1, float* disp,
                      const PostParams& pp, hipStream_t s, int nf = 1, long long fs_in = 0,
                      long long fs_out = 0, const HarrisParams* harris = nullptr);
int launch_median_f32(const float* in, int H, int W, float* out, hipStream_t s);
int launch_post_m16(const int16_t* in, long long n, float* disp, const PostParams& pp, hipStream_t s);
int launch_post(const float* disp, int n, const PostParams& pp, hipStream_t s);
int launch_post_lut(const PostParams& pp, int m0, int n, int step, float* lut_a, uint8_t* lut_u8,
                    float* lut_b, hipStream_t s);

}
```

stereovision_amd/csrc/sv_match.hip:

```cpp
#include "sv_match_packs.h"

namespace sv {
namespace {

int seg_mult(int kind, int r) {
    static const int sm4 = env_int("SV_SAD4_SEG", 1, 8);
    if (kind != COST_SAD4) return 4;
    if (sm4) return sm4;
    return (2 * r - 2 + 3) / 4 <= 2 ? 4 : 2;
}
__host__ __device__ constexpr bool hi_keys(int cost, int r) { return cost == COST_SAD4 && r <= 5; }
template <int COST, int ND, int NW>
__device__ __forceinline__ void ccol(const Pk<NW>& l, const Pk<NW>& r, uint32_t* v) {
    if constexpr (COST == COST_SAD) {
        uint32_t a = 0u;
#pragma unroll
        for (int i = 0; i < ND; ++i) a = __builtin_amdgcn_sad_u8(l.w[i], r.w[i], a);
        v[0] = a;
    } else if constexpr (COST == COST_SAD4) {
        constexpr int NC = NW - 4;
        uint32_t s = 0u;
#pragma unroll
        for (int i = 0; i < NC; ++i) s = __builtin_amdgcn_sad_u8(l.w[i], r.w[i], s);
#pragma unroll
// ... 92 lines not shown
    }
    if constexpr (LPG == 64) {
#pragma unroll
        for (int i = 0; i < N; ++i)
            v[i] = min(v[i], (uint32_t)__builtin_amdgcn_update_dpp(-1, (int)v[i], 0x143, 0xC, 0xF, false));
    }
}

__device__ __forceinline__ void reduce_scatter16(uint32_t (&v)[16], int l) {
#define SV_RS_STEP(HALF, BIT, CTRL)                                                            \
    {                                                                                          \
        const bool hi = (l & (BIT)) != 0;                                                      \
        _Pragma("unroll") for (int k = 0; k < (HALF); ++k) {                                   \
            const uint32_t send = hi ? v[k] : v[k + (HALF)];                                   \
            const uint32_t keep = hi ? v[k + (HALF)] : v[k];                                   \
            v[k] = min(keep, (uint32_t)__builtin_amdgcn_update_dpp(0u, (int)send, CTRL, 0xF, 0xF, false)); \
        }                                                                                      \
    }
    SV_RS_STEP(8, 8, 0x140)
    SV_RS_STEP(4, 4, 0x141)
    SV_RS_STEP(2, 2, 0x1B)
    SV_RS_STEP(1, 1, 0xB1)
#undef SV_RS_STEP
}
template <int COST, int ND> struct Occ {
    static constexpr int W = COST == COST_SAD4 ? 2 : (COST == COST_SAD || ND <= 3) ? 3 : 2;
};

template <int COST, int ND, int DPL>
__global__ __launch_bounds__((64 * PackCfg<COST, ND>::WPB), (Occ<COST, ND>::W)) void k_match(MatchParams a) {
    constexpr int NW = PackCfg<COST, ND>::NW;
    constexpr int ROWS = PackCfg<COST, ND>::ROWS;
    extern __shared__ __attribute__((aligned(16))) uint4 smem[];
    if (blockIdx.z) {
        a.L += blockIdx.z * a.fs_in;
        a.R += blockIdx.z * a.fs_in;
        a.out += blockIdx.z * a.fs_out;
        if constexpr (COST == COST_HOG) {
            a.HL += blockIdx.z * a.fs_hist;
            a.HR += blockIdx.z * a.fs_hist;
        }
    }
    const int lane = threadIdx.x & 63;
    const int wid = PackCfg<COST, ND>::WPB == 1 ? 0 : (int)(threadIdx.x >> 6);
    const int LPG = a.lpg;
    const int S = seg_width(LPG, DPL, a.segm);
    const int WC = wave_cols(LPG, DPL, a.segm);
    const int r = a.r;
    const int W2 = 2 * r + 1;
    SV_MATCH_REGIONS(WC, LPG, DPL, r)
    using P = PackCfg<COST, ND>;
    uint4* wbase = reinterpret_cast<uint4*>(reinterpret_cast<char*>(smem) + (size_t)wid * (NL + NRphys) * P::SLOT_BYTES);
    typename P::CT* cbase = reinterpret_cast<typename P::CT*>(wbase + (size_t)(NL + NRphys) * P::QX);
    const PackOut<COST, ND> Lw{wbase, cbase};
    const PackOut<COST, ND> Rw{wbase + (size_t)NL * P::QX, cbase + NL};
    const PackPtr<COST, ND> Lp{Lw.x, Lw.c};
    const PackPtr<COST, ND> Rp{Rw.x, Rw.c};

    const int y = a.row0 + ((int)blockIdx.y * PackCfg<COST, ND>::WPB + wid) * ROWS;
    const int yc = min(y, a.row1 - 1);
    const int xw = a.X0 + (int)blockIdx.x * WC;
    const int cL0 = xw - 3 * r - 1;
    const int cR0 = cL0 - a.minD - (LPG * DPL - 1);

    build_all_packs<COST, ND, DPL>(a, yc, cL0, NL, cR0, NRlog, c0, Lw, Rw, lane);

    if (blockIdx.x == 0) {
        const int16_t inv = (int16_t)((a.minD - 1) * 16);
#pragma unroll
        for (int q = 0; q < ROWS; ++q) {
            if (y + q >= a.row1) break;
            int16_t* orow = a.out + (size_t)(y + q) * a.opitch;
            for (int x = lane; x < a.X0; x += 64) orow[x] = inv;
            for (int x = a.X1 + lane; x < a.W; x += 64) orow[x] = inv;
        }
    }
    __syncthreads();
    if (y >= a.row1) return;

    const int g = lane >> a.lpg_log2;
    const int l = lane & (LPG - 1);
    const int sl = l ^ (((lane >> 4) & 1) << 3);
    const int xs = xw + g * S;
    const int iL0 = g * S + 2 * r + 1;
    const int iR0 = g * S + 2 * r + (LPG - sl) * DPL;
    const uint32_t dmask = (1u << a.dbits) - 1u;
    const int dbits = a.dbits;
    const int j = l - (LPG - 16);

    uint32_t mk[DPL];
    uint32_t h[DPL][ROWS], bk[ROWS][DPL];
#pragma unroll
    for (int k = 0; k < DPL; ++k) {
        const int idx = sl * DPL + k;
        mk[k] = idx < a.D ? (uint32_t)idx : 0xFFFFFFFFu;
#pragma unroll
        for (int q = 0; q < ROWS; ++q) h[k][q] = idx < a.D ? (uint32_t)idx : a.pad_key | (uint32_t)idx;
    }

    for (int t = 0; t < W2; ++t) {
        const Pk<NW> L = ld<COST, ND>(Lp + (iL0 + t));
#pragma unroll
        for (int k = 0; k < DPL; ++k) {
            uint32_t vn[ROWS];
            ccol<COST, ND, NW>(L, ld<COST, ND>(Rp + rslot(iR0 + t - k, c0, DPL)), vn);
            if constexpr (COST == COST_HOG) h[k][0] = (vn[0] << dbits) | mk[k];
            else {
#pragma unroll
                for (int q = 0; q < ROWS; ++q) h[k][q] += vn[q] << dbits;
            }
        }
    }
    {
        const bool emit0 = j == 0 && xs < a.X1;
#pragma unroll
        for (int q = 0; q < ROWS; ++q) {
            uint32_t b = 0xFFFFFFFFu;
#pragma unroll
            for (int k = 0; k < DPL; ++k) b = min(b, h[k][q]);
            if (LPG == 16) reduce_batch<16, 1>(&b);
            else if (LPG == 32) reduce_batch<32, 1>(&b);
            else reduce_batch<64, 1>(&b);
            if (emit0 && y + q < a.row1)
                a.out[(size_t)(y + q) * a.opitch + xs] = key_disp16(b, dmask, a.minD);
        }
    }

    const int phi = (DPL - W2 % DPL) % DPL;
    const int cut = DPL - phi;
    const int iN = iR0 + W2;
    Pk<NW> rn[DPL], ro[DPL];
#pragma unroll
    for (int s = 1; s < DPL; ++s) {
        rn[s] = ld<COST, ND>(Rp + rslot(iN - (DPL - s), c0, DPL));
        if constexpr (COST != COST_HOG) ro[s] = ld<COST, ND>(Rp + rslot(iR0 - (DPL - s), c0, DPL));
    }
    const PackPtr<COST, ND> rn0 = Rp + rslot(iN, c0, DPL);
    const PackPtr<COST, ND> ro0 = Rp + rslot(iR0, c0, DPL);
    const PackPtr<COST, ND> ln0 = Lp + (iL0 + W2);
    const PackPtr<COST, ND> lo0 = Lp + iL0;
    const int T = (S - 1 + DPL - 1) / DPL * DPL;

    for (int t0 = 0, c = 0; t0 < T; t0 += DPL, ++c) {
        match_chunk<COST, ND, DPL>(cut, dbits, rn0 + c * (DPL + 1), ro0 + c * (DPL + 1), ln0 + t0, lo0 + t0, rn,
                                   ro, h, mk, bk);
        if constexpr (ROWS * DPL == 16 || ROWS * DPL == 32) {
            if (LPG == 16) {
#pragma unroll
                for (int half = 0; half < ROWS * DPL / 16; ++half) {
                    uint32_t v[16];
#pragma unroll
                    for (int i = 0; i < 16; ++i) v[i] = bk[(16 * half + i) / DPL][i % DPL];
                    reduce_scatter16(v, l);
                    const int q = (16 * half) / DPL + l / DPL, e = t0 + l % DPL + 1, x = xs + e;
                    if (e < S && x < a.X1 && y + q < a.row1)
                        a.out[(size_t)(y + q) * a.opitch + x] = key_disp16(v[0], dmask, a.minD);
                }
                continue;
            }
        }
        if constexpr (ROWS * DPL == 8) {
            uint32_t v[8];
#pragma unroll
            for (int i = 0; i < 8; ++i) v[i] = bk[i / DPL][i % DPL];
            reduce_scatter8_bm(v, lane & 15);
            uint32_t key = v[0];
            if (LPG >= 32) {
                const auto p = __builtin_amdgcn_permlane16_swap(key, key, false, false);
                key = min(p[0], p[1]);
            }
            if (LPG == 64) {
                const auto p = __builtin_amdgcn_permlane32_swap(key, key, false, false);
                key = min(p[0], p[1]);
            }
            const int i = (l >> 1) & 7, q = i / DPL, e = t0 + i % DPL + 1, x = xs + e;
            if (l < 16 && (l & 1) == 0 && e < S && x < a.X1 && y + q < a.row1)
                a.out[(size_t)(y + q) * a.opitch + x] = key_disp16(key, dmask, a.minD);
            continue;
        }
        const int e = t0 + j + 1;
        const int x = xs + e;
        const bool emit = j >= 0 && j < DPL && e < S && x < a.X1;
        if (LPG == 16) reduce_batch<16, ROWS * DPL>(&bk[0][0]);
        else if (LPG == 32) reduce_batch<32, ROWS * DPL>(&bk[0][0]);
        else reduce_batch<64, ROWS * DPL>(&bk[0][0]);
#pragma unroll
        for (int q = 0; q < ROWS; ++q) {
            uint32_t v = bk[q][0];
#pragma unroll
            for (int u = 1; u < DPL; ++u) v = (j == u) ? bk[q][u] : v;
            if (emit && y + q < a.row1)
                a.out[(size_t)(y + q) * a.opitch + x] = key_disp16(v, dmask, a.minD);
        }
    }
}
__global__ void k_fill_i16(int16_t* out, int opitch, int H, int W, int16_t v) {
    const int x = blockIdx.x * blockDim.x + threadIdx.x;
    const int y = blockIdx.y;
    if (x < W && y < H) out[(size_t)y * opitch + x] = v;
}

template <int COST, int ND, int DPL>
int launch_one(const MatchParams& a, size_t lds, hipStream_t s) {
    auto fn = k_match<COST, ND, DPL>;
    if (lds > 65536) {
        hipError_t e = hipFuncSetAttribute((const void*)fn, hipFuncAttributeMaxDynamicSharedMemorySize, (int)lds);
        if (e != hipSuccess) return (int)e;
    }
    const int wc = wave_cols(a.lpg, DPL, a.segm);
    const int rows_per_block = PackCfg<COST, ND>::WPB * PackCfg<COST, ND>::ROWS;
    dim3 grid((a.X1 - a.X0 + wc - 1) / wc, (a.row1 - a.row0 + rows_per_block - 1) / rows_per_block,
              a.nf > 1 ? a.nf : 1);
    hipLaunchKernelGGL(fn, grid, dim3(64 * PackCfg<COST, ND>::WPB), lds, s, a);
    return (int)hipGetLastError();
}

template <int COST, int ND>
int launch_dpl(const MatchParams& a, const MatchPlan& p, size_t lds, hipStream_t s) {
    switch (p.dpl) {
        case 4: return launch_one<COST, ND, 4>(a, lds, s);
        case 6: return launch_one<COST, ND, 6>(a, lds, s);
        case 8: return launch_one<COST, ND, 8>(a, lds, s);
    }
    return (int)hipErrorInvalidValue;
}

template <int COST>
int launch_nd(const MatchParams& a, const MatchPlan& p, size_t lds, hipStream_t s) {
    if constexpr (COST == COST_HOG) {
        return launch_dpl<COST, 5>(a, p, lds, s);
    } else if constexpr (COST == COST_SAD4) {
        switch (p.ndw) {
            case 2: return launch_dpl<COST, 2>(a, p, lds, s);
            case 3: return launch_dpl<COST, 3>(a, p, lds, s);
            case 4: return launch_dpl<COST, 4>(a, p, lds, s);
            case 5: return launch_dpl<COST, 5>(a, p, lds, s);
            case 6: return launch_dpl<COST, 6>(a, p, lds, s);
            case 7: return launch_dpl<COST, 7>(a, p, lds, s);
        }
        return (int)hipErrorInvalidValue;
    } else {
        switch (p.ndw) {
            case 1: return launch_dpl<COST, 1>(a, p, lds, s);
            case 2: return launch_dpl<COST, 2>(a, p, lds, s);
            case 3: return launch_dpl<COST, 3>(a, p, lds, s);
            case 4: return launch_dpl<COST, 4>(a, p, lds, s);
        }
        return (int)hipErrorInvalidValue;
    }
}

}

uint64_t max_cost(int win, int cost) {
    return cost == COST_SAD ? (uint64_t)win * win * 255
         : cost == COST_SSD ? (uint64_t)win * win * 255 * 255
                            : (uint64_t)9 * win * win * 255;
}

int plan_match(int num_disp, int win, int cost, MatchPlan* plan) {
    static const int menu[][2] = {{4, 16}, {6, 16}, {8, 16}, {6, 32}, {8, 32}, {6, 64}, {8, 64}};
    if (num_disp <= 0 || win < 1 || (win & 1) == 0 || win > 15) return -22;
    if (cost != COST_SAD && cost != COST_SSD && cost != COST_HOG) return -22;
    int i = 0;
    for (; i < 7; ++i)
        if (menu[i][0] * menu[i][1] >= num_disp) break;
    if (i == 7) return -22;
    plan->dpl = menu[i][0];
    plan->lpg = menu[i][1];
    const int kind = kind_of(cost, win);
    plan->ndw = kind == COST_HOG ? 5 : kind == COST_SAD4 ? win / 2
              : (win + 3) / 4;
    int n = plan->dpl * plan->lpg - 1, bits = 0;
    while (n > 0) { ++bits; n >>= 1; }
    plan->dbits = bits < 1 ? 1 : bits;
    if (hi_keys(kind, win / 2)) plan->dbits = 16;
    const uint64_t cmax = max_cost(win, cost);
    const bool over = (cmax << plan->dbits) >= (1ull << 32) ||
                      (num_disp < plan->dpl * plan->lpg && cost != COST_HOG &&
                       ((2 * cmax + 2) << plan->dbits) >= (1ull << 32));
    plan->mfma_only = 0;
    if (over) {
        if (!ssd_mfma(cost, win, num_disp)) return -34;
        plan->mfma_only = 1;
    }
    return 0;
}

size_t match_lds_bytes(const MatchPlan& p, int r, int cost) {
    const int kind = kind_of(cost, 2 * r + 1);
    const int wpb = kind == COST_SAD4 ? 1 : 4;
    SV_MATCH_REGIONS(wave_cols(p.lpg, p.dpl, seg_mult(kind, r)), p.lpg, p.dpl, r)
    return (size_t)wpb * (NL + NRphys) * pack_shape(kind, p.ndw).slot_bytes;
}

int launch_fill_i16(int16_t* out, int opitch, int H, int W, int16_t v, hipStream_t s) {
    if (H <= 0 || W <= 0) return 0;
    hipLaunchKernelGGL(k_fill_i16, dim3((W + 255) / 256, H), dim3(256), 0, s, out, opitch, H, W, v);
    return (int)hipGetLastError();
}

int launch_match(const MatchParams& a, const MatchPlan& p, int cost, hipStream_t s) {
    if (a.row1 <= a.row0) return 0;
    if (a.X1 <= a.X0) {
        for (int z = 0; z < (a.nf > 1 ? a.nf : 1); ++z) {
            int e = launch_fill_i16(a.out + z * a.fs_out + (size_t)a.row0 * a.opitch, a.opitch,
                                    a.row1 - a.row0, a.W, (int16_t)((a.minD - 1) * 16), s);
            if (e) return e;
        }
        return 0;
    }
    if (ssd_mfma_fits(a, cost)) return launch_ssd_mfma(a, s);
    if (p.mfma_only) return (int)hipErrorInvalidValue;
    const int e = launch_match_ring(a, cost, s);
    if (e >= 0) return e;
    const size_t lds = match_lds_bytes(p, a.r, cost);
    if (lds > 160 * 1024) return (int)hipErrorInvalidValue;
    MatchParams b = a;
    b.segm = seg_mult(kind_of(cost, a.win), a.r);
    switch (kind_of(cost, a.win)) {
        case COST_SAD: return launch_nd<COST_SAD>(b, p, lds, s);
        case COST_SAD4: return launch_nd<COST_SAD4>(b, p, lds, s);
        case COST_SSD: return launch_nd<COST_SSD>(b, p, lds, s);
        case COST_HOG: return launch_nd<COST_HOG>(b, p, lds, s);
    }
    return (int)hipErrorInvalidValue;
}

}
```

stereovision_amd/csrc/sv_match_ring.hip:

```cpp
#include "sv_match_packs.h"
#include "sv_xcd.h"

#include <cstdio>

namespace sv {
namespace {

typedef unsigned short u16x2 __attribute__((ext_vector_type(2)));
__device__ __forceinline__ uint32_t pk_add16(uint32_t a, uint32_t b) {
    return __builtin_bit_cast(uint32_t, __builtin_bit_cast(u16x2, a) + __builtin_bit_cast(u16x2, b));
}

typedef uint32_t lds_u32x4 __attribute__((ext_vector_type(4), may_alias));

template <int R, int LPGT, bool DEFER, bool KEYS, bool SSD = false, bool LDSMIN = false>
__global__ __launch_bounds__(64, 2) void k_match_ring(MatchParams a) {
    using P = PackCfg<COST_SAD4, R>;
    constexpr int NW = P::NW, NC = P::NC, W2 = 2 * R + 1;
    static_assert(!LDSMIN || (LPGT == 32 && R <= 5), "the LDS fold is laid out for two 32-lane groups of 32-bit keys");
    constexpr bool PK = R >= 6;
    static_assert(P::SPLIT && (P::CW == 3) == PK, "ring kind expects split packs (20 B for r 2..3, 24 B for r 4..5, 28 B for r 6..7)");
    extern __shared__ __attribute__((aligned(16))) uint4 smem[];
    int bx, by, bz;
    xcd_tile(a.xcd_map != 0, bx, by, bz);
    if (bz) {
        a.L += bz * a.fs_in;
        a.R += bz * a.fs_in;
        a.out += bz * a.fs_out;
        if constexpr (KEYS) a.keys += bz * a.fs_out;
    }
    const int lane = threadIdx.x;
    constexpr int LPG = LPGT;
    const int S = a.segm;
    constexpr int M = W2 + 1;
    constexpr int U = M % 4 == 0 ? M : M % 2 == 0 ? 2 * M : 4 * M;
    constexpr int NCH = U / 4;
    SV_RING_GEOM(LPG, S, R)
    constexpr int c0 = RING_C0;
    const int nit = (Tn + U - 1) / U;
    const int e0 = (nit * U - Tn) >> 2;
    uint4* wbase = smem + ring_scratch_bytes(LDSMIN) / 16;
    typename P::CT* cbase = reinterpret_cast<typename P::CT*>(wbase + (size_t)slots);
    const PackOut<COST_SAD4, R> Lw{wbase + RING_PAD_F, cbase + RING_PAD_F};
    const PackOut<COST_SAD4, R> Rw{wbase + NL + RING_PAD_F + RING_PAD_M, cbase + NL + RING_PAD_F + RING_PAD_M};
    const PackPtr<COST_SAD4, R> Lp{Lw.x, Lw.c};
    const PackPtr<COST_SAD4, R> Rp{Rw.x, Rw.c};

    const int y = a.row0 + by * 4;
    const int yc = min(y, a.row1 - 1);
    const int xw = a.X0 + bx * WC;
    const int cL0 = xw - R;
    const int cR0 = cL0 - a.minD - (4 * LPG - 1);
    build_ring_packs<R, 3, RG_DPL>(a, yc, cL0, NL, cR0, NRlog, c0, Lw, Rw, lane);

    if (!KEYS && bx == 0 && !a.margins_done) {
        const int16_t inv = (int16_t)((a.minD - 1) * 16);
#pragma unroll
        for (int q = 0; q < 4; ++q) {
            if (y + q >= a.row1) break;
            int16_t* orow = a.out + (size_t)(y + q) * a.opitch;
            for (int x = lane; x < a.X0; x += 64) orow[x] = inv;
            for (int x = a.X1 + lane; x < a.W; x += 64) orow[x] = inv;
        }
    }
    __syncthreads();
    if (y >= a.row1) return;

    const int g = lane / LPG;
    const int l = lane & (LPG - 1);
    const int xs = xw + g * S;
    const int dl = PK ? min(4 * l, a.D - 4) : 4 * l;
    const int iR0 = g * S + 4 * (LPG - 1) - dl + 3;
    constexpr int RQ = PK ? 2 : 4;
    uint32_t h[RG_DPL][RQ], lab[RG_DPL];
#pragma unroll
    for (int k = 0; k < RG_DPL; ++k) {
        const int idx = 4 * l + k;
        const uint32_t base = PK ? 0u : idx < a.D ? (uint32_t)idx : (SSD ? a.pad_key : 0x8000u << 16) | (uint32_t)idx;
        lab[k] = (uint32_t)idx;
#pragma unroll
        for (int q = 0; q < RQ; ++q) h[k][q] = base;
    }
    uint32_t ring[M][RG_DPL][RQ];
#pragma unroll
    for (int s = 0; s < M; ++s)
#pragma unroll
        for (int k = 0; k < RG_DPL; ++k)
#pragma unroll
            for (int q = 0; q < RQ; ++q) asm volatile("" : "=v"(ring[s][k][q]));
    Pk<NW> rn[RG_DPL];
#pragma unroll
    for (int s = 1; s < RG_DPL; ++s) rn[RG_DPL - s] = ld<COST_SAD4, R, true>(Rp + rslot(iR0 - s, c0, RG_DPL));
    PackPtr<COST_SAD4, R> rb = Rp + (rslot(iR0, c0, RG_DPL) - e0 * (RG_DPL + 1));
    PackPtr<COST_SAD4, R> lb = Lp + (g * S - 4 * e0);
    constexpr bool LPF = R != 5;
    Pk<NW> Lnext = ld<COST_SAD4, R, true>(lb + 4 * e0);
    const int jq = (lane >> 2) & 3, ju = (lane >> 1) & 1;
    constexpr bool join2 = LPG >= 32;
    int pofs = 0;
    if (join2 && !LDSMIN) {
        const auto p = __builtin_amdgcn_permlane16_swap((uint32_t)lane, (uint32_t)lane + 64u, false, false);
        pofs = (max(p[0], p[1]) < 64u) ? 0 : 2;
    }
    const int eq = LDSMIN ? lane >> 4 : jq;
    const int exs = LDSMIN ? xw + ((lane >> 2) & 1) * S : xs;
    const int eb = (LDSMIN ? ((lane >> 3) & 1) + 2 * (lane & 1) : ju + pofs) - 2 * R;
    constexpr int OB = KEYS ? 4 : 2;
    const int ooff = OB * ((y + eq) * a.opitch + exs + eb);
    const auto orsrc = KEYS ? __builtin_amdgcn_make_buffer_rsrc(a.keys, 0, 0x7FFFFFFF, 0x00020000)
                            : __builtin_amdgcn_make_buffer_rsrc(a.out, 0, 0x7FFFFFFF, 0x00020000);
    const int emax = (LDSMIN ? (lane & 2) == 0 && y + eq < a.row1
                             : (l & 1) == 0 && l < (join2 ? 32 : 16) && y + jq < a.row1)
                         ? max(0, min(S, a.X1 - exs)) : 0;

    auto emit_key = [&](uint32_t key, int tt) {
        const int off = (unsigned)(tt + eb) < (unsigned)emax ? ooff + OB * tt : (int)0x80000000u;
        if constexpr (KEYS) __builtin_amdgcn_raw_buffer_store_b32(key, orsrc, off, 0, 0);
        else __builtin_amdgcn_raw_buffer_store_b16(
            (uint16_t)key_disp16(key, SSD ? (1u << a.dbits) - 1u : 0xFFFFu, a.minD), orsrc, off, 0, 0);
    };
    auto join_pairs = [&](uint32_t kA_, uint32_t kB_) {
        auto p = __builtin_amdgcn_permlane16_swap(kA_, kB_, false, false);
        uint32_t key = min(p[0], p[1]);
        if (LPG == 64) {
            p = __builtin_amdgcn_permlane32_swap(key, key, false, false);
            key = min(p[0], p[1]);
        }
        return key;
    };
    auto join_rows = [&](uint32_t key) {
        if (LPG >= 32) {
            const auto p = __builtin_amdgcn_permlane16_swap(key, key, false, false);
            key = min(p[0], p[1]);
        }
        if (LPG == 64) {
            const auto p = __builtin_amdgcn_permlane32_swap(key, key, false, false);
            key = min(p[0], p[1]);
        }
        return key;
    };
    uint32_t dv[8], kA = 0xFFFFFFFFu;
    int tprev = -(1 << 24);
#pragma unroll
    for (int i = 0; i < 8; ++i) dv[i] = 0xFFFFFFFFu;
    [[maybe_unused]] uint32_t* const scr = reinterpret_cast<uint32_t*>(smem);
    [[maybe_unused]] const uint32_t scr_m0 = __builtin_amdgcn_readfirstlane(
        (uint32_t)(uintptr_t)(__attribute__((address_space(3))) uint32_t*)scr);
    [[maybe_unused]] const lds_u32x4* const sra = reinterpret_cast<const lds_u32x4*>(scr + 8 * lane + 4 * ((lane >> 3) & 1));
    [[maybe_unused]] const lds_u32x4* const srb = reinterpret_cast<const lds_u32x4*>(scr + 8 * lane + 4 * (1 - ((lane >> 3) & 1)));
    auto lds_fold = [&](const lds_u32x4& p, const lds_u32x4& s) {
        uint32_t m = min(min(p.x, p.y), p.z);
        m = min(min(m, p.w), s.x);
        m = min(min(m, s.y), s.z);
        m = min(m, s.w);
        m = min(m, (uint32_t)__builtin_amdgcn_update_dpp(0u, (int)m, 0xB1, 0xF, 0xF, false));
        return min(m, (uint32_t)__builtin_amdgcn_update_dpp(0u, (int)m, 0x4E, 0xF, 0xF, false));
    };
    [[maybe_unused]] const bool pairB = (lane & 1) != 0;

    constexpr int NZ = 2 * R - 4 * (2 * R / 4) + 1;
    auto chunk = [&](auto warm_c, const int ch, const int t0) __attribute__((always_inline)) {
            constexpr bool WARM = decltype(warm_c)::value;
            [[maybe_unused]] uint32_t bk[4][2];
#pragma unroll
            for (int u = 0; u < 4; ++u) {
                const int slot = (4 * ch + u) % M, oslot = (4 * ch + u + 1) % M;
                rn[u] = ld<COST_SAD4, R, true>(rb + (ch * (RG_DPL + 1) + u));
                const Pk<NW> Lc = LPF ? Lnext : ld<COST_SAD4, R, true>(lb + (4 * ch + u));
                if constexpr (LPF) Lnext = ld<COST_SAD4, R, true>(lb + (4 * ch + u + 1));
                lds_u32x4 fa{}, fb{};
                if constexpr (LDSMIN && !WARM) {
                    if ((u & 1) == 0) { fa = *sra; fb = *srb; }
                }
                uint32_t sqL[4];
                if constexpr (SSD) {
                    uint32_t sc = 0u;
#pragma unroll
                    for (int i = 0; i < NC; ++i) sc = __builtin_amdgcn_udot4(Lc.w[i], Lc.w[i], sc, false);
#pragma unroll
                    for (int q = 0; q < 4; ++q)
                        sqL[q] = __builtin_amdgcn_udot4(Lc.w[NC + q], Lc.w[NC + q], sc, false) << a.dbits;
                }
#pragma unroll
                for (int kk = 0; kk < RG_DPL; ++kk) {
                    const int k = RG_DPL - 1 - kk;
                    const Pk<NW>& Rk = rn[(u - k) & 3];
                    if constexpr (PK) {
                        uint32_t cn = 0u;
#pragma unroll
                        for (int i = 0; i < NC; ++i) cn = __builtin_amdgcn_sad_u8(Lc.w[i], Rk.w[i], cn);
                        cn |= cn << 16;
#pragma unroll
                        for (int j = 0; j < 2; ++j) {
                            const uint32_t c = __builtin_amdgcn_sad_hi_u8(
                                Lc.w[NC + 2 * j + 1], Rk.w[NC + 2 * j + 1],
                                __builtin_amdgcn_sad_u8(Lc.w[NC + 2 * j], Rk.w[NC + 2 * j], cn));
                            if constexpr (!WARM) sad_u32_acc(h[k][j], ring[oslot][k][j], c);
                            else h[k][j] = pk_add16(h[k][j], c);
                            ring[slot][k][j] = c;
                        }
                    } else if constexpr (SSD) {
                        uint32_t cn = 0u, sr = 0u;
#pragma unroll
                        for (int i = 0; i < NC; ++i) {
                            cn = __builtin_amdgcn_udot4(Lc.w[i], Rk.w[i], cn, false);
                            sr = __builtin_amdgcn_udot4(Rk.w[i], Rk.w[i], sr, false);
                        }
#pragma unroll
                        for (int q = 0; q < 4; ++q) {
                            const uint32_t lr = __builtin_amdgcn_udot4(Lc.w[NC + q], Rk.w[NC + q], cn, false);
                            const uint32_t rr = __builtin_amdgcn_udot4(Rk.w[NC + q], Rk.w[NC + q], sr, false);
                            const uint32_t t = (rr << a.dbits) + sqL[q];
                            const uint32_t c = (uint32_t)__mul24((int)lr, -(2 << a.dbits)) + t;
                            if constexpr (WARM) h[k][q] += c;
                            else sad_u32_acc(h[k][q], ring[oslot][k][q], c);
                            ring[slot][k][q] = c;
                        }
                    } else {
                        uint32_t cn = 0u;
#pragma unroll
                        for (int i = 0; i < NC; ++i) cn = __builtin_amdgcn_sad_hi_u8(Lc.w[i], Rk.w[i], cn);
#pragma unroll
                        for (int q = 0; q < 4; ++q) {
                            const uint32_t c = __builtin_amdgcn_sad_hi_u8(Lc.w[NC + q], Rk.w[NC + q], cn);
                            if constexpr (!WARM) sad_u32_acc(h[k][q], ring[oslot][k][q], c);
                            else h[k][q] += c;
                            ring[slot][k][q] = c;
                        }
                    }
                }
                if constexpr (WARM) {
                    __builtin_amdgcn_sched_barrier(0);
                    continue;
                }
#pragma unroll
                for (int q = 0; q < 4; ++q) {
                    uint32_t kq[RG_DPL];
#pragma unroll
                    for (int k = 0; k < RG_DPL; ++k)
                        kq[k] = !PK ? h[k][q] : (q & 1) ? (h[k][q >> 1] & 0xFFFF0000u) | lab[k] : (h[k][q >> 1] << 16) | lab[k];
                    bk[q][u & 1] = min(min(kq[0], kq[1]), min(kq[2], kq[3]));
                }
                if constexpr (LDSMIN) {
                    if (u == 2) {
                        kA = lds_fold(fa, fb);
                    } else if (u == 0) {
                        const uint32_t kB = lds_fold(fa, fb);
                        emit_key(pairB ? kB : kA, tprev);
                        tprev = t0;
                    }
                }
                __builtin_amdgcn_sched_barrier(0);
                if constexpr (LDSMIN) {
                    if (u & 1) {
                        asm volatile("s_mov_b32 m0, %8\n\t"
                                     "s_nop 0\n\t"
                                     "ds_write_addtid_b32 %0\n\t"
                                     "ds_write_addtid_b32 %1 offset:256\n\t"
                                     "ds_write_addtid_b32 %2 offset:512\n\t"
                                     "ds_write_addtid_b32 %3 offset:768\n\t"
                                     "ds_write_addtid_b32 %4 offset:1024\n\t"
                                     "ds_write_addtid_b32 %5 offset:1280\n\t"
                                     "ds_write_addtid_b32 %6 offset:1536\n\t"
                                     "ds_write_addtid_b32 %7 offset:1792\n\t"
                                     :
                                     : "v"(bk[0][0]), "v"(bk[0][1]), "v"(bk[1][0]), "v"(bk[1][1]), "v"(bk[2][0]),
                                       "v"(bk[2][1]), "v"(bk[3][0]), "v"(bk[3][1]), "s"(scr_m0)
                                     : "memory", "m0");
                        __builtin_amdgcn_fence(__ATOMIC_SEQ_CST, "wavefront");
                    }
                    continue;
                }
                if (DEFER && u == 3) {
#pragma unroll
                    for (int i = 0; i < 8; ++i) dv[i] = bk[i >> 1][i & 1];
                } else if (DEFER && u == 1) {
                    uint32_t v[8];
#pragma unroll
                    for (int i = 0; i < 8; ++i) v[i] = bk[i >> 1][i & 1];
                    reduce_scatter8_bm(v, lane & 15);
                    reduce_scatter8_bm(dv, lane & 15);
                    if (join2) {
                        emit_key(join_pairs(kA, dv[0]), tprev);
                        kA = v[0];
                    } else {
                        emit_key(join_rows(dv[0]), tprev + 2);
                        emit_key(join_rows(v[0]), t0);
                    }
                    tprev = t0;
                } else if (u & 1) {
                    uint32_t v[8];
#pragma unroll
                    for (int i = 0; i < 8; ++i) v[i] = bk[i >> 1][i & 1];
                    reduce_scatter8_bm(v, lane & 15);
                    if (join2) {
                        if (u == 1) kA = v[0];
                        else emit_key(join_pairs(kA, v[0]), t0);
                    } else {
                        emit_key(join_rows(v[0]), t0 + u - 1);
                    }
                }
            }
            if constexpr (WARM) {
                if (t0 + 7 >= 2 * R) {
#pragma unroll
                    for (int i = 0; i < NZ; ++i)
#pragma unroll
                        for (int k = 0; k < RG_DPL; ++k)
#pragma unroll
                            for (int q = 0; q < RQ; ++q) ring[(4 * ch + 5 + i) % M][k][q] = 0u;
                }
            }
    };
    constexpr int NWARM = 2 * R / 4;
#pragma unroll
    for (int e = 0; e < NCH; ++e) {
        if (e != e0) continue;
#pragma unroll
        for (int i = 0; i < NWARM; ++i) chunk(std::true_type{}, e + i, 4 * i);
    }
    for (int it = 0, t0 = -4 * e0; it < nit; ++it) {
#pragma unroll
        for (int ch = 0; ch < NCH; ++ch, t0 += 4) {
            if (t0 < 4 * NWARM) continue;
            chunk(std::false_type{}, ch, t0);
        }
        rb = rb + NCH * (RG_DPL + 1);
        lb = lb + U;
    }
    if constexpr (LDSMIN) {
        const uint32_t kB = lds_fold(*sra, *srb);
        emit_key(pairB ? kB : kA, tprev);
    } else if (DEFER) {
        reduce_scatter8_bm(dv, lane & 15);
        if (join2) emit_key(join_pairs(kA, dv[0]), tprev);
        else emit_key(join_rows(dv[0]), tprev + 2);
    }
}

bool ring_kind(int cost, int win, int num_disp) {
    static const bool on = env_flag("SV_RING", true);
    return on && kind_of(cost, win) == COST_SAD4 && win >= 5 && num_disp <= 256 &&
           (win <= 11 || (win <= 15 && num_disp % 4 == 0));
}
int ring_lpg(int num_disp) { return num_disp <= 64 ? 16 : num_disp <= 128 ? 32 : 64; }
bool ring_ldsmin(int lpg, int r, bool keys, bool ssd) {
    static const bool on = env_flag("SV_RING_LDSMIN", true);
    return on && lpg == 32 && r == 4 && !keys && !ssd;
}
size_t ring_lds_bytes(int lpg, int seg, int r, bool ldsmin) {
    SV_RING_GEOM(lpg, seg, r)
    return (size_t)slots * pack_shape(COST_SAD4, r).slot_bytes + ring_scratch_bytes(ldsmin);
}
int ring_seg(int lpg, int r, int band, bool ldsmin) {
    static const int env = [] {
        const int v = env_int("SV_RING_SEG", 8, 1024);
        return v % 4 == 0 ? v : 0;
    }();
    if (env) return env;
    const int G = 64 / lpg;
    int best = 8;
    long long best_cost = -1;
    for (int S = 8; S <= 1024; S += 4) {
        if (S > 8 && ring_lds_bytes(lpg, S, r, ldsmin) > 20 * 1024) break;
        SV_RING_GEOM(lpg, S, r)
        const long long cost = (long long)((band + G * S - 1) / (G * S)) * Tn;
        if (best_cost < 0 || cost <= best_cost) { best = S; best_cost = cost; }
    }
    return best;
}

template <int R, int LPG, bool KEYS, bool SSD>
int launch_ring_rl(const MatchParams& a, size_t lds, bool ldsmin, hipStream_t s) {
    static const bool defer = env_flag("SV_RING_DEFER", true);
    void (*fn)(MatchParams);
    if constexpr (SSD) fn = k_match_ring<R, LPG, R != 5, false, true>;
    else if constexpr (KEYS) fn = k_match_ring<R, LPG, R != 5, true>;
    else fn = (defer && R != 5) ? k_match_ring<R, LPG, R != 5, false> : k_match_ring<R, LPG, false, false>;
    if constexpr (R == 4 && LPG == 32 && !KEYS && !SSD) {
        if (ldsmin) fn = k_match_ring<R, LPG, false, false, false, true>;
    }
    if (lds > 65536) {
        hipError_t e = hipFuncSetAttribute((const void*)fn, hipFuncAttributeMaxDynamicSharedMemorySize, (int)lds);
        if (e != hipSuccess) return (int)e;
    }
    const int wc = (64 / a.lpg) * a.segm;
    dim3 grid((a.X1 - a.X0 + wc - 1) / wc, (a.row1 - a.row0 + 3) / 4, a.nf > 1 ? a.nf : 1);
    static const bool occ = env_flag("SV_RING_OCC", false);
    if (occ) {
        int nb = -1;
        (void)hipOccupancyMaxActiveBlocksPerMultiprocessor(&nb, (const void*)fn, 64, lds);
        std::fprintf(stderr, "k_match_ring r=%d lpg=%d ldsmin=%d seg=%d lds=%zu B: %d waves/CU\n", R, LPG,
                     (int)ldsmin, a.segm, lds, nb);
    }
    static const bool xcd = env_flag("SV_XCD_MAP", true);
    MatchParams b = a;
    b.xcd_map = xcd ? 1 : 0;
    hipLaunchKernelGGL(fn, grid, dim3(64), lds, s, b);
    return (int)hipGetLastError();
}
template <int R, bool KEYS, bool SSD = false>
int launch_ring_r(const MatchParams& a, size_t lds, bool ldsmin, hipStream_t s) {
    switch (a.lpg) {
        case 16: return launch_ring_rl<R, 16, KEYS, SSD>(a, lds, ldsmin, s);
        case 32: return launch_ring_rl<R, 32, KEYS, SSD>(a, lds, ldsmin, s);
        case 64: return launch_ring_rl<R, 64, KEYS, SSD>(a, lds, ldsmin, s);
    }
    return (int)hipErrorInvalidValue;
}

template <bool KEYS, bool SSD = false>
int launch_ring(const MatchParams& a0, hipStream_t s) {
    MatchParams a = a0;
    a.lpg = ring_lpg(a.D);
    a.lpg_log2 = a.lpg == 16 ? 4 : a.lpg == 32 ? 5 : 6;
    a.dbits = SSD ? a.lpg_log2 + 2 : 16;
    if (SSD) a.pad_key = (uint32_t)((max_cost(a.win, COST_SSD) + 1) << a.dbits);
    const bool ldsmin = ring_ldsmin(a.lpg, a.r, KEYS, SSD);
    a.segm = ring_seg(a.lpg, a.r, a.X1 - a.X0, ldsmin);
    const size_t lds = ring_lds_bytes(a.lpg, a.segm, a.r, ldsmin);
    if (lds > 160 * 1024) return (int)hipErrorInvalidValue;
    if constexpr (SSD) {
        switch (a.r) {
            case 2: return launch_ring_r<2, false, true>(a, lds, ldsmin, s);
            case 3: return launch_ring_r<3, false, true>(a, lds, ldsmin, s);
            case 4: return launch_ring_r<4, false, true>(a, lds, ldsmin, s);
        }
        return (int)hipErrorInvalidValue;
    } else {
        switch (a.r) {
            case 2: return launch_ring_r<2, KEYS>(a, lds, ldsmin, s);
            case 3: return launch_ring_r<3, KEYS>(a, lds, ldsmin, s);
            case 4: return launch_ring_r<4, KEYS>(a, lds, ldsmin, s);
            case 5: return launch_ring_r<5, KEYS>(a, lds, ldsmin, s);
            case 6: return launch_ring_r<6, KEYS>(a, lds, ldsmin, s);
            case 7: return launch_ring_r<7, KEYS>(a, lds, ldsmin, s);
        }
        return (int)hipErrorInvalidValue;
    }
}

__device__ __forceinline__ int16_t merge_px(uint32_t ka, uint32_t kb, int x, int X0, int X1, int minD) {
    const uint32_t k = min(ka, kb + 256u);
    return (int16_t)(x >= X0 && x < X1 ? ((int)(k & 0xFFFFu) + minD) * 16 : (minD - 1) * 16);
}
__global__ __launch_bounds__(256) void k_merge_ring_keys(const uint32_t* __restrict__ ka,
                                                         const uint32_t* __restrict__ kb, int16_t* __restrict__ out,
                                                         int opitch, long long fs_out, int row0, int W, int X0, int X1,
                                                         int minD, int vec) {
    const int x = 4 * (int)(blockIdx.x * 256 + threadIdx.x);
    if (x >= W) return;
    const size_t i = (size_t)blockIdx.z * fs_out + (size_t)(row0 + (int)blockIdx.y) * opitch + x;
    if (vec && x + 4 <= W) {
        const uint4 a = *reinterpret_cast<const uint4*>(ka + i);
        const uint4 b = *reinterpret_cast<const uint4*>(kb + i);
        const uint32_t lo = (uint16_t)merge_px(a.x, b.x, x, X0, X1, minD) |
                            ((uint32_t)(uint16_t)merge_px(a.y, b.y, x + 1, X0, X1, minD) << 16);
        const uint32_t hi = (uint16_t)merge_px(a.z, b.z, x + 2, X0, X1, minD) |
                            ((uint32_t)(uint16_t)merge_px(a.w, b.w, x + 3, X0, X1, minD) << 16);
        *reinterpret_cast<uint2*>(out + i) = make_uint2(lo, hi);
        return;
    }
    for (int q = 0; q < 4 && x + q < W; ++q) out[i + q] = merge_px(ka[i + q], kb[i + q], x + q, X0, X1, minD);
}

}

bool ring_ssd(int cost, int win, int num_disp) {
    if (cost != COST_SSD || win < 5 || win > 9 || num_disp < 1 || num_disp > 256) return false;
    if (!ring_kind(COST_SAD, win, num_disp)) return false;
    const int lpg = ring_lpg(num_disp), dbits = (lpg == 16 ? 4 : lpg == 32 ? 5 : 6) + 2;
    const uint64_t cmax = max_cost(win, COST_SSD);
    const uint64_t top = num_disp < 4 * lpg ? (2 * cmax + 2) << dbits : (cmax << dbits) + (uint64_t)(4 * lpg);
    return top < (1ull << 32);
}
bool ring_split(int cost, int win, int num_disp) {
    return num_disp > 256 && num_disp <= 512 && ring_kind(cost, win, 256) && ring_kind(cost, win, num_disp - 256);
}
long long ring_split_elems(int nf, long long fs_out, int row1, int opitch) {
    return ((long long)(nf > 1 ? nf - 1 : 0) * fs_out + (long long)(row1 + 3) * opitch + 64 + 3) & ~3LL;
}

int launch_match_ring(const MatchParams& a, int cost, hipStream_t s) {
    const bool ring_fits = 2LL * ((long long)(a.row1 + 3) * a.opitch + a.W + 64) < 0x7FFFFFFFLL;
    if (ring_kind(cost, a.win, a.D) && ring_fits) return launch_ring<false>(a, s);
    if (ring_ssd(cost, a.win, a.D) && ring_fits) return launch_ring<false, true>(a, s);
    if (ring_split(cost, a.win, a.D) && a.keys) {
        if (4LL * ((long long)(a.row1 + 3) * a.opitch + a.W + 64) >= 0x7FFFFFFFLL) return (int)hipErrorInvalidValue;
        MatchParams pa = a, pb = a;
        pa.D = 256;
        pb.minD = a.minD + 256;
        pb.D = a.D - 256;
        pb.keys = a.keys + a.keys_stride;
        int e = launch_ring<true>(pa, s);
        if (!e) e = launch_ring<true>(pb, s);
        if (e) return e;
        const int nf = a.nf > 1 ? a.nf : 1;
        const long long fso = nf > 1 ? a.fs_out : 0LL;
        const int vec = (a.opitch % 4 == 0 && fso % 4 == 0 && a.keys_stride % 4 == 0 &&
                         ((uintptr_t)a.out & 7) == 0 && ((uintptr_t)a.keys & 15) == 0) ? 1 : 0;
        hipLaunchKernelGGL(k_merge_ring_keys, dim3((a.W + 1023) / 1024, a.row1 - a.row0, nf), dim3(256), 0, s, pa.keys,
                           pb.keys, a.out, a.opitch, fso, a.row0, a.W, a.X0, a.X1, a.minD, vec);
        return (int)hipGetLastError();
    }
    return -1;
}

}
```

stereovision_amd/csrc/sv_median.hip:

```cpp
#include <type_traits>
#include "sv_harris_wave.h"
#include "sv_median_net.h"

namespace sv {
namespace {

struct PostVals { float a, b; uint8_t u; };

__device__ __forceinline__ PostVals post_vals(const PostParams& pp, float d) {
    PostVals o{0.0f, 0.0f, 0};
    if (pp.mode == POST_DEPTH) {
        const float fxb = (float)(700 * 0.08);
        const float den = d + (float)1e-6;
        const float depth = fxb / den;
        float dc = depth < pp.minf ? pp.minf : depth;
        dc = dc > pp.maxf ? pp.maxf : dc;
        const bool valid = (d > pp.min_disp_global) && (dc >= pp.minf) && (dc <= pp.maxf);
        o.a = valid ? dc : 0.0f;
        float t = dc - pp.minf;
        t = t / pp.rangef;
        t = t * 255.0f;
        o.u = (uint8_t)(int)t;
    } else if (pp.mode == POST_SCALED) {
        const float lo = (float)pp.min_disp, hi = (float)(pp.min_disp + pp.num_disp - 1);
        float c = d < lo ? lo : d;
        c = c > hi ? hi : c;
        float t = c - lo;
        t = t / (float)pp.num_disp;
        t = t * 255.0f;
        o.u = (uint8_t)(int)t;
        o.a = (float)o.u;
        o.b = (d > (float)(pp.min_disp + 1) && d < hi) ? 1.0f : 0.0f;
    }
    return o;
}

template <typename T>
__device__ __forceinline__ T& at(T* base, uint32_t i) {
    using B = typename std::conditional<std::is_const<T>::value, const char, char>::type;
    return *reinterpret_cast<T*>(reinterpret_cast<B*>(base) + (uint32_t)(i * (uint32_t)sizeof(T)));
}
template <typename T>
__device__ __forceinline__ T& at(T* base, size_t i) { return base[i]; }

template <typename I>
__device__ __forceinline__ void store_post(const PostParams& pp, I i, const PostVals& o) {
    at(pp.out_a, i) = o.a;
    at(pp.out_u8, i) = o.u;
    if (pp.mode == POST_SCALED) at(pp.out_b, i) = o.b;
}

__device__ __forceinline__ void post_one(const PostParams& pp, size_t i, float d) {
    if (pp.mode == POST_NONE) return;
    store_post(pp, i, post_vals(pp, d));
}

typedef short s2 __attribute__((ext_vector_type(2)));
constexpr int MT_W = 64, MT_H = 8;
constexpr int MQ_W = 128, MQ_H = 16;

__device__ __forceinline__ s2 as_s2(uint32_t u) { return __builtin_bit_cast(s2, u); }

__device__ __forceinline__ s2 net_min(s2 a, s2 b) { return __builtin_elementwise_min(a, b); }
__device__ __forceinline__ s2 net_max(s2 a, s2 b) { return __builtin_elementwise_max(a, b); }
__device__ __forceinline__ float net_min(float a, float b) { return fminf(a, b); }
__device__ __forceinline__ float net_max(float a, float b) { return fmaxf(a, b); }
template <typename T, int N, int M>
__device__ __forceinline__ void apply_net(T* v, const unsigned char (&net)[N][M]) {
#pragma unroll
    for (int c = 0; c < N; ++c) {
        const int a = net[c][0], b = net[c][1], use = M == 3 ? net[c][M - 1] : 3;
        const T lo = net_min(v[a], v[b]), hi = net_max(v[a], v[b]);
        if (use & 1) v[a] = lo;
        if (use & 2) v[b] = hi;
    }
}

__device__ __forceinline__ PostVals lut_entry(const PostParams& pp, uint32_t li) {
    PostVals o;
    o.a = at(pp.lut_a, li);
    o.u = at(pp.lut_u8, li);
    o.b = pp.mode == POST_SCALED ? at(pp.lut_b, li) : 0.0f;
    return o;
}
__device__ __forceinline__ PostVals post_median(const PostParams& pp, int mv) {
    const uint32_t dm = (uint32_t)(mv - pp.lut_m0);
    const uint32_t li = dm >> pp.lut_shift;
    if (li < (uint32_t)pp.lut_n && (dm & ((1u << pp.lut_shift) - 1u)) == 0) return lut_entry(pp, li);
    return post_vals(pp, (float)mv / 16.0f);
}
__device__ __forceinline__ PostVals post_median_whole(const PostParams& pp, int mv) {
    return lut_entry(pp, ((uint32_t)(mv - pp.lut_m0) >> 4) & (uint32_t)(kLutWholeSpan - 1));
}

__global__ __launch_bounds__(256) void k_post_m16(const int16_t* __restrict__ in, long long n,
                                                  float* __restrict__ disp, PostParams pp) {
    const long long i0 = ((long long)blockIdx.x * 256 + threadIdx.x) * 8;
    if (i0 >= n) return;
    const bool vec = i0 + 8 <= n && ((((uintptr_t)in) & 15) | (((uintptr_t)disp | (uintptr_t)pp.out_a |
                                                                  (uintptr_t)pp.out_b) & 15) |
                                     ((uintptr_t)pp.out_u8 & 7)) == 0;
    if (vec) {
        const uint4 raw = *reinterpret_cast<const uint4*>(in + i0);
        const uint32_t w[4] = {raw.x, raw.y, raw.z, raw.w};
        int mv[8];
#pragma unroll
        for (int q = 0; q < 4; ++q) {
            mv[2 * q] = (int)(int16_t)(w[q] & 0xFFFFu);
            mv[2 * q + 1] = (int)(int16_t)(w[q] >> 16);
        }
        if (disp) {
            float4* d = reinterpret_cast<float4*>(disp + i0);
            d[0] = make_float4((float)mv[0] / 16.0f, (float)mv[1] / 16.0f, (float)mv[2] / 16.0f, (float)mv[3] / 16.0f);
            d[1] = make_float4((float)mv[4] / 16.0f, (float)mv[5] / 16.0f, (float)mv[6] / 16.0f, (float)mv[7] / 16.0f);
        }
        if (pp.mode == POST_NONE) return;
        PostVals o[8];
#pragma unroll
        for (int q = 0; q < 8; ++q) o[q] = post_median(pp, mv[q]);
        float4* a = reinterpret_cast<float4*>(pp.out_a + i0);
        a[0] = make_float4(o[0].a, o[1].a, o[2].a, o[3].a);
        a[1] = make_float4(o[4].a, o[5].a, o[6].a, o[7].a);
        uint32_t u[2] = {0u, 0u};
#pragma unroll
        for (int q = 0; q < 8; ++q) u[q >> 2] |= (uint32_t)o[q].u << (8 * (q & 3));
        *reinterpret_cast<uint2*>(pp.out_u8 + i0) = make_uint2(u[0], u[1]);
        if (pp.mode == POST_SCALED) {
            float4* b = reinterpret_cast<float4*>(pp.out_b + i0);
            b[0] = make_float4(o[0].b, o[1].b, o[2].b, o[3].b);
            b[1] = make_float4(o[4].b, o[5].b, o[6].b, o[7].b);
        }
        return;
    }
    for (long long i = i0; i < i0 + 8 && i < n; ++i) {
        const int mv = (int)in[i];
        if (disp) disp[i] = (float)mv / 16.0f;
        if (pp.mode == POST_NONE) continue;
        store_post(pp, (size_t)i, post_median(pp, mv));
    }
}

template <int HF, bool WH>
__global__ __launch_bounds__(256) void k_median_i16(const int16_t* __restrict__ in, int H, int W,
                                                    int row0, int row1, float* __restrict__ disp,
                                                    PostParams pp, long long fs_in, long long fs_out,
                                                    HarrisParams hp) {
    if (HF != 0 && (int)blockIdx.x >= hp.mbx) {
        const int w = (int)(blockIdx.x - hp.mbx) * 4 + (int)(threadIdx.x >> 6);
        const int y0 = row0 + (int)blockIdx.y * MQ_H;
        if constexpr (HF == 2) {
            const int x0 = w * 248;
            if (x0 < W && y0 < row1)
                harris_wave4<MQ_H, 4>(hp.g + blockIdx.z * hp.fs_in, H, W, hp.pitch, hp.out + blockIdx.z * hp.fs_out,
                                      x0, y0, threadIdx.x & 63);
        } else {
            const int x0 = w * 60;
            if (x0 < W && y0 < row1)
                harris_wave<MQ_H, 4>(hp.g + blockIdx.z * hp.fs_in, H, W, hp.pitch, hp.out + blockIdx.z * hp.fs_out,
                                     x0, y0, threadIdx.x & 63);
        }
        return;
    }
    constexpr int TC = MQ_W + 4, TR = MQ_H + 2;
    __shared__ uint32_t t2[TR][TC];
    __shared__ __attribute__((aligned(8))) uint32_t srt[MQ_H / 4][4][TC];
    if (blockIdx.z) {
        in += blockIdx.z * fs_in;
        const long long o = blockIdx.z * fs_out;
        if (disp) disp += o;
        if (pp.out_a) pp.out_a += o;
        if (pp.out_u8) pp.out_u8 += o;
        if (pp.out_b) pp.out_b += o;
        if (pp.out_bgr) pp.out_bgr += 3 * o;
        if (pp.out_m16) pp.out_m16 += o;
        if (pp.out_d8) pp.out_d8 += o;
    }
    const int x0 = blockIdx.x * MQ_W, y0 = row0 + blockIdx.y * MQ_H;
    {
        const int c = (int)(threadIdx.x & (MQ_W - 1)), g = (int)(threadIdx.x / MQ_W);
        constexpr int G = 256 / MQ_W;
        static_assert(TR % G == 0, "row groups must tile the pair rows");
        const uint32_t cx = (uint32_t)clampi(x0 - 2 + c, 0, W - 1);
        if (y0 >= 2 && y0 + TR - 1 <= H - 1) {
            uint32_t off = (uint32_t)(y0 - 2 + g) * W + cx;
            const uint32_t two = 2u * (uint32_t)W, step = (uint32_t)G * W;
#pragma unroll
            for (int k = 0; k < TR / G; ++k) {
                const uint16_t a = (uint16_t)at(in, off);
                const uint16_t b = (uint16_t)at(in, off + two);
                t2[g + G * k][c] = (uint32_t)a | ((uint32_t)b << 16);
                off += step;
            }
        } else {
#pragma unroll
            for (int k = 0; k < TR / G; ++k) {
                const int r = g + G * k;
                const uint16_t a = (uint16_t)at(in, (uint32_t)clampi(y0 - 2 + r, 0, H - 1) * W + cx);
                const uint16_t b = (uint16_t)at(in, (uint32_t)clampi(y0 + r, 0, H - 1) * W + cx);
                t2[r][c] = (uint32_t)a | ((uint32_t)b << 16);
            }
        }
        if (threadIdx.x < 4 * TR) {
            const int r = (int)(threadIdx.x >> 2), ce = MQ_W + (int)(threadIdx.x & 3);
            const uint32_t cxe = (uint32_t)clampi(x0 - 2 + ce, 0, W - 1);
            const uint16_t a = (uint16_t)at(in, (uint32_t)clampi(y0 - 2 + r, 0, H - 1) * W + cxe);
            const uint16_t b = (uint16_t)at(in, (uint32_t)clampi(y0 + r, 0, H - 1) * W + cxe);
            t2[r][ce] = (uint32_t)a | ((uint32_t)b << 16);
        }
    }
    __syncthreads();
    const int tx = 2 * (int)(threadIdx.x & 63), tb = 4 * (int)(threadIdx.x >> 6);
    {
        auto sort_col = [&](int g4, int c) {
            s2 w[4];
#pragma unroll
            for (int i = 0; i < 4; ++i) w[i] = as_s2(t2[g4 + 1 + i][c]);
            apply_net(w, SV_SORT4_NET);
#pragma unroll
            for (int i = 0; i < 4; ++i) srt[g4 >> 2][i][c] = __builtin_bit_cast(uint32_t, w[i]);
        };
        sort_col(tb, tx);
        sort_col(tb, tx + 1);
        if (threadIdx.x < 16) sort_col(4 * (threadIdx.x >> 2), MQ_W + (threadIdx.x & 3));
    }
    __syncthreads();

    s2 cm[16], own[2][4];
#pragma unroll
    for (int i = 0; i < 4; ++i) {
        const uint2 p0 = *reinterpret_cast<const uint2*>(&srt[tb >> 2][i][tx]);
        const uint2 p1 = *reinterpret_cast<const uint2*>(&srt[tb >> 2][i][tx + 2]);
        const uint2 p2 = *reinterpret_cast<const uint2*>(&srt[tb >> 2][i][tx + 4]);
        own[0][i] = as_s2(p0.x);
        cm[0 * 4 + i] = as_s2(p0.y);
        cm[1 * 4 + i] = as_s2(p1.x);
        cm[2 * 4 + i] = as_s2(p1.y);
        cm[3 * 4 + i] = as_s2(p2.x);
        own[1][i] = as_s2(p2.y);
    }
    apply_net(cm, SV_SEL16H_NET);
    s2 cw[2][6];
#pragma unroll
    for (int w = 0; w < 2; ++w) {
        s2 z[14];
#pragma unroll
        for (int k = 0; k < 10; ++k) z[k] = cm[SV_SEL16H_OUT[k]];
#pragma unroll
        for (int k = 0; k < 4; ++k) z[10 + k] = own[w][k];
        apply_net(z, SV_MRG14_NET);
#pragma unroll
        for (int k = 0; k < 6; ++k) cw[w][k] = z[SV_MRG14_OUT[k]];
    }
    uint32_t mp[4];
#pragma unroll
    for (int h = 0; h < 2; ++h) {
        s2 q[6];
        {
            const uint2 p0 = *reinterpret_cast<const uint2*>(&t2[tb + 5 * h][tx]);
            const uint2 p1 = *reinterpret_cast<const uint2*>(&t2[tb + 5 * h][tx + 2]);
            const uint2 p2 = *reinterpret_cast<const uint2*>(&t2[tb + 5 * h][tx + 4]);
            q[0] = as_s2(p0.x); q[1] = as_s2(p0.y); q[2] = as_s2(p1.x);
            q[3] = as_s2(p1.y); q[4] = as_s2(p2.x); q[5] = as_s2(p2.y);
        }
        s2 sc[4] = {q[1], q[2], q[3], q[4]};
        apply_net(sc, SV_SORT4_NET);
        s2 m[2];
#pragma unroll
        for (int w = 0; w < 2; ++w) {
            s2 u[5] = {sc[0], sc[1], sc[2], sc[3], w ? q[5] : q[0]};
#pragma unroll
            for (int k = 3; k >= 0; --k) {
                const s2 lo = __builtin_elementwise_min(u[k], u[k + 1]);
                u[k + 1] = __builtin_elementwise_max(u[k], u[k + 1]);
                u[k] = lo;
            }
            s2 r = cw[w][5];
#pragma unroll
            for (int i = 0; i < 5; ++i) r = __builtin_elementwise_min(r, __builtin_elementwise_max(cw[w][i], u[4 - i]));
            m[w] = r;
        }
        const uint32_t a0 = __builtin_bit_cast(uint32_t, m[0]), a1 = __builtin_bit_cast(uint32_t, m[1]);
        mp[h] = (a0 & 0xFFFFu) | (a1 << 16);
        mp[h + 2] = (a0 >> 16) | (a1 & 0xFFFF0000u);
    }
    static_assert(sizeof(srt) >= MQ_H * (MQ_W / 2) * sizeof(uint32_t), "med must fit in srt");
    auto med = reinterpret_cast<uint32_t (*)[MQ_W / 2]>(&srt[0][0][0]);
    __syncthreads();
    med[tb][tx >> 1] = mp[0];
    med[tb + 1][tx >> 1] = mp[1];
    med[tb + 2][tx >> 1] = mp[2];
    med[tb + 3][tx >> 1] = mp[3];
    __syncthreads();
    auto post = [&](int mv) { return WH ? post_median_whole(pp, mv) : post_median(pp, mv); };
    const bool vec = (W & 3) == 0 &&
                     (((uintptr_t)disp | (uintptr_t)pp.out_a | (uintptr_t)pp.out_b) & 15) == 0 &&
                     (((uintptr_t)pp.out_u8 | (uintptr_t)pp.out_bgr | (uintptr_t)pp.out_d8) & 3) == 0 &&
                     ((uintptr_t)pp.out_m16 & 7) == 0;
#pragma unroll
    for (int pass = 0; pass < 2; ++pass) {
        const int r = (int)(threadIdx.x >> 5) + 8 * pass, c4 = (int)(threadIdx.x & 31) * 4;
        const int y = y0 + r, x = x0 + c4;
        if (y >= row1 || x >= W) continue;
        const uint2 raw = *reinterpret_cast<const uint2*>(&med[r][c4 >> 1]);
        const int mv[4] = {(int)(int16_t)(raw.x & 0xFFFF), (int)(int16_t)(raw.x >> 16),
                           (int)(int16_t)(raw.y & 0xFFFF), (int)(int16_t)(raw.y >> 16)};
        const uint32_t i = (uint32_t)y * W + x;
        if (vec) {
            if (disp)
                at(reinterpret_cast<float4*>(disp), i >> 2) =
                    make_float4((float)mv[0] / 16.0f, (float)mv[1] / 16.0f, (float)mv[2] / 16.0f, (float)mv[3] / 16.0f);
            if (pp.out_m16) at(reinterpret_cast<uint2*>(pp.out_m16), i >> 2) = raw;
            if (pp.out_d8)
                at(reinterpret_cast<uint32_t*>(pp.out_d8), i >> 2) =
                    (uint32_t)(uint8_t)((mv[0] >> 4) - pp.d8_base) | ((uint32_t)(uint8_t)((mv[1] >> 4) - pp.d8_base) << 8) |
                    ((uint32_t)(uint8_t)((mv[2] >> 4) - pp.d8_base) << 16) |
                    ((uint32_t)(uint8_t)((mv[3] >> 4) - pp.d8_base) << 24);
            if (pp.mode == POST_NONE) continue;
            PostVals o[4];
#pragma unroll
            for (int q = 0; q < 4; ++q) o[q] = post(mv[q]);
            at(reinterpret_cast<float4*>(pp.out_a), i >> 2) = make_float4(o[0].a, o[1].a, o[2].a, o[3].a);
            at(reinterpret_cast<uint32_t*>(pp.out_u8), i >> 2) =
                (uint32_t)o[0].u | ((uint32_t)o[1].u << 8) | ((uint32_t)o[2].u << 16) | ((uint32_t)o[3].u << 24);
            if (pp.mode == POST_SCALED)
                at(reinterpret_cast<float4*>(pp.out_b), i >> 2) = make_float4(o[0].b, o[1].b, o[2].b, o[3].b);
            if (pp.out_bgr) {
                const uint32_t c0 = pp.cmap[o[0].u], c1 = pp.cmap[o[1].u], c2 = pp.cmap[o[2].u],
                               c3 = pp.cmap[o[3].u];
                uint32_t* d = &at(reinterpret_cast<uint32_t*>(pp.out_bgr), 3 * (i >> 2));
                d[0] = c0 | (c1 << 24);
                d[1] = (c1 >> 8) | (c2 << 16);
                d[2] = (c2 >> 16) | (c3 << 8);
            }
            continue;
        }
#pragma unroll
        for (int q = 0; q < 4; ++q) {
            if (x + q >= W) break;
            if (disp) at(disp, i + q) = (float)mv[q] / 16.0f;
            if (pp.out_m16) at(pp.out_m16, i + q) = (int16_t)mv[q];
            if (pp.out_d8) at(pp.out_d8, i + q) = (uint8_t)((mv[q] >> 4) - pp.d8_base);
            if (pp.mode == POST_NONE) continue;
            const PostVals o = post(mv[q]);
            store_post(pp, i + q, o);
            if (pp.out_bgr) {
                const uint32_t c = pp.cmap[o.u];
                uint8_t* d = &at(pp.out_bgr, 3 * (i + q));
                d[0] = (uint8_t)c;
                d[1] = (uint8_t)(c >> 8);
                d[2] = (uint8_t)(c >> 16);
            }
        }
    }
}

__global__ __launch_bounds__(256) void k_median_f32(const float* __restrict__ in, int H, int W,
                                                    float* __restrict__ out) {
    __shared__ float tile[MT_H + 4][MT_W + 4];
    const int x0 = blockIdx.x * MT_W, y0 = blockIdx.y * MT_H;
    for (int i = threadIdx.x; i < (MT_H + 4) * (MT_W + 4); i += 256) {
        const int ty = i / (MT_W + 4), tx = i % (MT_W + 4);
        tile[ty][tx] = in[(size_t)clampi(y0 - 2 + ty, 0, H - 1) * W + clampi(x0 - 2 + tx, 0, W - 1)];
    }
    __syncthreads();
    const int tx = threadIdx.x % MT_W, pr = threadIdx.x / MT_W;
#pragma unroll
    for (int h = 0; h < 2; ++h) {
        float v[25];
#pragma unroll
        for (int j = 0; j < 5; ++j)
#pragma unroll
            for (int i = 0; i < 5; ++i) v[j * 5 + i] = tile[2 * pr + h + j][tx + i];
        apply_net(v, SV_MED25_NET);
        const int x = x0 + tx, y = y0 + 2 * pr + h;
        if (x < W && y < H) out[(size_t)y * W + x] = v[SV_MED25_OUT];
    }
}

__global__ void k_post(const float* __restrict__ disp, int n, PostParams pp) {
    const int i = blockIdx.x * blockDim.x + threadIdx.x;
    if (i < n) post_one(pp, (size_t)i, disp[i]);
}

__global__ void k_post_lut(PostParams pp, int m0, int n, int step) {
    const int i = blockIdx.x * blockDim.x + threadIdx.x;
    if (i < n) post_one(pp, (size_t)i, (float)(m0 + i * step) / 16.0f);
}

}

int launch_median_i16(const int16_t* in, int H, int W, int row0, int row1, float* disp,
                      const PostParams& pp, hipStream_t s, int nf, long long fs_in, long long fs_out,
                      const HarrisParams* harris) {
    if (row1 <= row0 || nf <= 0) return 0;
    if ((long long)H * W >= (1LL << 30)) return (int)hipErrorInvalidValue;
    HarrisParams hp{};
    int hbx = 0;
    if (harris && harris->g) {
        hp = *harris;
        static const bool med4 = env_flag("SV_HARRIS_MED4", true);
        hp.form = (med4 && W >= 256) ? 1 : 0;
        hbx = hp.form ? ((W + 247) / 248 + 3) / 4 : ((W + 59) / 60 + 3) / 4;
    }
    hp.mbx = (W + MQ_W - 1) / MQ_W;
    const bool wh = pp.lut_unchecked && pp.mode != POST_NONE && pp.lut_shift == 4 && pp.lut_n > 0 &&
                    pp.lut_cap >= kLutWholeSpan;
    void (*fn)(const int16_t*, int, int, int, int, float*, PostParams, long long, long long, HarrisParams) =
        wh ? (hbx == 0 ? k_median_i16<0, true> : hp.form ? k_median_i16<2, true> : k_median_i16<1, true>)
           : (hbx == 0 ? k_median_i16<0, false> : hp.form ? k_median_i16<2, false> : k_median_i16<1, false>);
    hipLaunchKernelGGL(fn, dim3(hp.mbx + hbx, (row1 - row0 + MQ_H - 1) / MQ_H, nf),
                       dim3(256), 0, s, in, H, W, row0, row1, disp, pp, fs_in, fs_out, hp);
    return (int)hipGetLastError();
}

int launch_post_m16(const int16_t* in, long long n, float* disp, const PostParams& pp, hipStream_t s) {
    if (n <= 0) return 0;
    const long long blocks = (n + 8 * 256 - 1) / (8 * 256);
    if (blocks > 0x7FFFFFFFLL) return (int)hipErrorInvalidValue;
    hipLaunchKernelGGL(k_post_m16, dim3((unsigned)blocks), dim3(256), 0, s, in, n, disp, pp);
    return (int)hipGetLastError();
}

int launch_median_f32(const float* in, int H, int W, float* out, hipStream_t s) {
    hipLaunchKernelGGL(k_median_f32, dim3((W + MT_W - 1) / MT_W, (H + MT_H - 1) / MT_H), dim3(256),
                       0, s, in, H, W, out);
    return (int)hipGetLastError();
}

int launch_post_lut(const PostParams& pp, int m0, int n, int step, float* lut_a, uint8_t* lut_u8,
                    float* lut_b, hipStream_t s) {
    if (n <= 0 || pp.mode == POST_NONE) return 0;
    PostParams q = pp;
    q.out_a = lut_a;
    q.out_u8 = lut_u8;
    q.out_b = lut_b;
    q.out_bgr = nullptr;
    q.out_m16 = nullptr;
    q.lut_n = 0;
    hipLaunchKernelGGL(k_post_lut, dim3((n + 255) / 256), dim3(256), 0, s, q, m0, n, step);
    return (int)hipGetLastError();
}

int launch_post(const float* disp, int n, const PostParams& pp, hipStream_t s) {
    if (n <= 0 || pp.mode == POST_NONE) return 0;
    hipLaunchKernelGGL(k_post, dim3((n + 255) / 256), dim3(256), 0, s, disp, n, pp);
    return (int)hipGetLastError();
}

}
```

Baseline: 32460.

## Write SAD ring disparities as u8 plane and median-filter from bytes

When the whole pipeline runs with the SAD matcher and the parameters allow it, the ring matcher stores a one-byte disparity index (offset by one) instead of a 16-bit fixed-point value. The median kernel is templated to read that u8 plane and rebuild the float, m16 and d8 outputs from the LUT base. This halves the intermediate disparity traffic between the match and median stages. It adds a separate scratch buffer with its own margin tracking and an env flag to turn it off. It only applies when num_disp is at most 255 and the LUT covers whole disparities.

```diff
diff --git a/stereovision_amd/csrc/sv_capi.cpp b/stereovision_amd/csrc/sv_capi.cpp
--- a/stereovision_amd/csrc/sv_capi.cpp
+++ b/stereovision_amd/csrc/sv_capi.cpp
@@ -158,15 +158,20 @@
 int enqueue_disparity(sv_ctx* c, const uint8_t* L, const uint8_t* R, int H, int W, int pitch,
                       int min_disp, int num_disp, int win, int cost, int row0, int row1,
                       int16_t* out, int opitch, hipStream_t s, int nf, long long fs_in,
-                      long long fs_out, bool track_margins) {
+                      long long fs_out, bool track_margins, uint8_t* out8) {
     sv::MatchPlan plan;
     int rc = check_match(H, W, min_disp, num_disp, win, cost, &plan);
     if (rc) return rc;
     if (row0 < 0) row0 = 0;
     if (row1 > H) row1 = H;
     if (row1 <= row0) return 0;
-    const sv_ctx::MarginKey had = c->d16_margins;
-    c->scratch_written(out);
+    if (out8 && (out || cost != SV_COST_SAD || out8 != c->d8.as<uint8_t>() || row0 != 0 || row1 != H))
+        return fail(SV_EINVAL, "the u8 plane takes whole frames of the SAD matcher");
+    sv_ctx::MarginKey& margins = out8 ? c->d8_margins : c->d16_margins;
+    const DevBuf& mbuf = out8 ? c->d8 : c->d16;
+    const sv_ctx::MarginKey had = margins;
+    if (out8) margins.valid = false;
+    else c->scratch_written(out);
     if (cost == SV_COST_SGBM) {
         if (row0 != 0 || row1 != H) return fail(SV_EINVAL, "SGBM cannot compute a row band (use frames)");
         return enqueue_sgbm(c, L, R, H, W, pitch, min_disp, num_disp, win, sgbm_reference_params(win), out, opitch,
@@ -194,6 +199,7 @@
     a.dbits = plan.dbits;
     a.pad_key = (uint32_t)((sv::max_cost(win, cost) + 1) << plan.dbits);
     a.out = out;
+    a.out8 = out8;
     a.opitch = opitch;
     a.nf = nf < 1 ? 1 : nf;
     a.fs_in = fs_in;
@@ -218,10 +224,10 @@
         a.keys_stride = ke;
     }
     sv_ctx::MarginKey key;
-    if (track_margins && out == c->d16.as<int16_t>() && row0 == 0 && row1 == H) {
+    if (track_margins && (out8 || out == c->d16.as<int16_t>()) && row0 == 0 && row1 == H) {
         key.valid = true;
-        key.p = c->d16.p;
-        key.gen = c->d16.gen;
+        key.p = mbuf.p;
+        key.gen = mbuf.gen;
         key.H = H;
         key.W = W;
         key.opitch = opitch;
@@ -234,7 +240,7 @@
         if (a.margins_done) key = had;
     }
     SV_LAUNCH(c, SV_K_MATCH, s, sv::launch_match(a, plan, cost, s));
-    if (key.valid) c->d16_margins = key;
+    if (key.valid) margins = key;
     return 0;
 }
 
@@ -528,7 +534,7 @@
                           &c->rmap1, &c->rmap2, &c->rdst[0], &c->rdst[1], &c->stats, &c->sel,
                           &c->sg_hsum, &c->sg_c, &c->sg_l, &c->sg_lt, &c->sg_band, &c->cc_parent,
                           &c->hist_copies, &c->cmap, &c->bgr, &c->m16,
-                          &c->cc_size, &c->sg_rec, &c->gm16, &c->keys, &c->lutw, &c->fuse, &c->flow};
+                          &c->cc_size, &c->sg_rec, &c->gm16, &c->keys, &c->lutw, &c->fuse, &c->flow, &c->d8};
         if (c->lut_ev) (void)hipEventDestroy(c->lut_ev);
         if (c->lutw_ev) (void)hipEventDestroy(c->lutw_ev);
         if (c->scr_ev) (void)hipEventDestroy(c->scr_ev);
@@ -582,9 +588,10 @@
     DevBuf* bufs[] = {&c->img[0], &c->img[1], &c->gray[0], &c->gray[1], &c->d16, &c->fa, &c->fb, &c->fc,
                       &c->u8, &c->harris, &c->hog[0], &c->hog[1], &c->fin, &c->sg_hsum, &c->sg_c,
                       &c->sg_l, &c->sg_lt, &c->sg_band, &c->sg_rec, &c->cc_parent, &c->cc_size, &c->m16,
-                      &c->gm16, &c->keys, &c->flow};
+                      &c->gm16, &c->keys, &c->flow, &c->d8};
     for (auto* b : bufs) b->release();
     c->d16_margins.valid = false;
+    c->d8_margins.valid = false;
     return 0;
 }
 
diff --git a/stereovision_amd/csrc/sv_capi_dev.cpp b/stereovision_amd/csrc/sv_capi_dev.cpp
--- a/stereovision_amd/csrc/sv_capi_dev.cpp
+++ b/stereovision_amd/csrc/sv_capi_dev.cpp
@@ -99,32 +99,55 @@
     hipStream_t s = pick(c, stream);
     SV_SCRATCH(c, s);
     const long long fs = (long long)H * W;
+    static const bool d8_on = sv::env_flag("SV_D8_PATH", true);
+    const int maxd = min_disp + num_disp;
+    const bool band = (maxd > 0 ? maxd : 0) < W + (min_disp < 0 ? min_disp : 0);
+    sv::PostParams pp;
+    float* disp = nullptr;
+    auto attach_outputs = [&]() -> int {
+        const int rc = map_out_post(c, out, min_disp, num_disp, cost, true, s, &pp, &disp);
+        if (rc) return rc;
+        pp.lut_unchecked = match && cost != SV_COST_SGBM && pp.lut_shift == 4 && pp.lut_m0 == (min_disp - 1) * 16 &&
+                           pp.lut_n == num_disp + 1;
+        return 0;
+    };
+    const bool attached = d8_on && stages == SV_STAGE_ALL && !d_disp16 && W % 4 == 0 && band &&
+                          sv::ring_out8(cost, win, num_disp, H, W, W);
+    bool use8 = false;
+    if (attached) {
+        const int rc = attach_outputs();
+        if (rc) return rc;
+        use8 = sv::median_u8_ok(pp);
+    }
     int16_t* d16 = d_disp16;
-    if (!d16) {
+    if (use8) {
+        SV_HIP(c->d8.ensure((size_t)n_frames * fs));
+    } else if (!d16) {
         SV_HIP(c->d16.ensure((size_t)n_frames * fs * sizeof(int16_t)));
         d16 = c->d16.as<int16_t>();
     }
     if (match) {
         const int rc = enqueue_disparity(c, d_left, d_right, H, W, pitch, min_disp, num_disp, win, cost, 0, H, d16, W,
-                                         s, n_frames, frame_stride, fs, !d_disp16);
+                                         s, n_frames, frame_stride, fs, !d_disp16, use8 ? c->d8.as<uint8_t>() : nullptr);
         if (rc) return rc;
     }
     if (!median) return 0;
-    sv::PostParams pp;
-    float* disp = nullptr;
-    int rc = map_out_post(c, out, min_disp, num_disp, cost, true, s, &pp, &disp);
-    if (rc) return rc;
-    pp.lut_unchecked = match && cost != SV_COST_SGBM && pp.lut_shift == 4 && pp.lut_m0 == (min_disp - 1) * 16 &&
-                       pp.lut_n == num_disp + 1;
+    if (!attached) {
+        const int rc = attach_outputs();
+        if (rc) return rc;
+    }
     const long long fin = n_frames > 1 ? frame_stride : 0;
+    auto launch_median = [&](const sv::HarrisParams* hp) {
+        return use8 ? sv::launch_median_u8(c->d8.as<uint8_t>(), H, W, 0, H, disp, pp, s, n_frames, fs, fs, hp)
+                    : sv::launch_median_i16(d16, H, W, 0, H, disp, pp, s, n_frames, fs, fs, hp);
+    };
     if (out->harris && (W < 8 || H < 8)) {
-        SV_LAUNCH(c, SV_K_MEDIAN, s, sv::launch_median_i16(d16, H, W, 0, H, disp, pp, s, n_frames, fs, fs));
+        SV_LAUNCH(c, SV_K_MEDIAN, s, launch_median(nullptr));
         SV_LAUNCH(c, SV_K_HARRIS, s, sv::launch_harris(d_left, H, W, pitch, out->harris, s, n_frames, fin, fs));
         return 0;
     }
     sv::HarrisParams hp{d_left, pitch, fin, out->harris, fs, 0, 0};
-    SV_LAUNCH(c, SV_K_MEDIAN, s,
-              sv::launch_median_i16(d16, H, W, 0, H, disp, pp, s, n_frames, fs, fs, out->harris ? &hp : nullptr));
+    SV_LAUNCH(c, SV_K_MEDIAN, s, launch_median(out->harris ? &hp : nullptr));
     return 0;
 }
 
diff --git a/stereovision_amd/csrc/sv_ctx.h b/stereovision_amd/csrc/sv_ctx.h
--- a/stereovision_amd/csrc/sv_ctx.h
+++ b/stereovision_amd/csrc/sv_ctx.h
@@ -113,6 +113,7 @@
     DevBuf m16;
     DevBuf gm16;
     DevBuf keys;
+    DevBuf d8;
     std::vector<float> hl_a, hl_b;
     std::vector<uint8_t> hl_u8;
     std::vector<HostEnt> hl_ent;
@@ -151,6 +152,7 @@
                    (o.nf <= 1 || fs_out == o.fs_out);
         }
     } d16_margins;
+    MarginKey d8_margins;
     void scratch_written(const void* out) {
         const char* b = static_cast<const char*>(d16.p);
         const char* o = static_cast<const char*>(out);
@@ -248,7 +250,7 @@
 int enqueue_disparity(sv_ctx* c, const uint8_t* L, const uint8_t* R, int H, int W, int pitch,
                       int min_disp, int num_disp, int win, int cost, int row0, int row1,
                       int16_t* out, int opitch, hipStream_t s, int nf = 1, long long fs_in = 0,
-                      long long fs_out = 0, bool track_margins = false);
+                      long long fs_out = 0, bool track_margins = false, uint8_t* out8 = nullptr);
 int attach_lut(sv_ctx* c, sv::PostParams& pp, hipStream_t s, bool whole = false);
 int attach_cmap(sv_ctx* c, sv::PostParams& pp, const uint8_t* table, uint8_t* d_bgr, hipStream_t s);
 sv::PostParams make_post(int mode, float minf, float maxf, float rangef, float mdg, int min_disp,
diff --git a/stereovision_amd/csrc/sv_internal.h b/stereovision_amd/csrc/sv_internal.h
--- a/stereovision_amd/csrc/sv_internal.h
+++ b/stereovision_amd/csrc/sv_internal.h
@@ -70,6 +70,7 @@
     uint32_t* keys;
     long long keys_stride;
     int margins_done;
+    uint8_t* out8;
 };
 
 int plan_match(int num_disp, int win, int cost, MatchPlan* plan);
@@ -82,6 +83,7 @@
 bool ssd_mfma_fits(const MatchParams& a, int cost);
 int launch_ssd_mfma(const MatchParams& a, hipStream_t s);
 long long ring_split_elems(int nf, long long fs_out, int row1, int opitch);
+bool ring_out8(int cost, int win, int num_disp, int row1, int opitch, int W);
 int launch_fill_i16(int16_t* out, int opitch, int H, int W, int16_t v, hipStream_t s);
 
 int launch_gray(const uint8_t* bgr, int H, int W, int pitch, uint8_t* gray, hipStream_t s);
@@ -335,6 +337,10 @@
 int launch_median_i16(const int16_t* in, int H, int W, int row0, int row1, float* disp,
                       const PostParams& pp, hipStream_t s, int nf = 1, long long fs_in = 0,
                       long long fs_out = 0, const HarrisParams* harris = nullptr);
+bool median_u8_ok(const PostParams& pp);
+int launch_median_u8(const uint8_t* in, int H, int W, int row0, int row1, float* disp, const PostParams& pp,
+                     hipStream_t s, int nf = 1, long long fs_in = 0, long long fs_out = 0,
+                     const HarrisParams* harris = nullptr);
 int launch_median_f32(const float* in, int H, int W, float* out, hipStream_t s);
 int launch_post_m16(const int16_t* in, long long n, float* disp, const PostParams& pp, hipStream_t s);
 int launch_post(const float* disp, int n, const PostParams& pp, hipStream_t s);
diff --git a/stereovision_amd/csrc/sv_match.hip b/stereovision_amd/csrc/sv_match.hip
--- a/stereovision_amd/csrc/sv_match.hip
+++ b/stereovision_amd/csrc/sv_match.hip
@@ -418,6 +418,11 @@
 
 int launch_match(const MatchParams& a, const MatchPlan& p, int cost, hipStream_t s) {
     if (a.row1 <= a.row0) return 0;
+    if (a.out8) {
+        if (a.X1 <= a.X0) return (int)hipErrorInvalidValue;
+        const int e = launch_match_ring(a, cost, s);
+        return e >= 0 ? e : (int)hipErrorInvalidValue;
+    }
     if (a.X1 <= a.X0) {
         for (int z = 0; z < (a.nf > 1 ? a.nf : 1); ++z) {
             int e = launch_fill_i16(a.out + z * a.fs_out + (size_t)a.row0 * a.opitch, a.opitch,
diff --git a/stereovision_amd/csrc/sv_match_ring.hip b/stereovision_amd/csrc/sv_match_ring.hip
--- a/stereovision_amd/csrc/sv_match_ring.hip
+++ b/stereovision_amd/csrc/sv_match_ring.hip
@@ -13,9 +13,10 @@
 
 typedef uint32_t lds_u32x4 __attribute__((ext_vector_type(4), may_alias));
 
-template <int R, int LPGT, bool DEFER, bool KEYS, bool SSD = false, bool LDSMIN = false>
+template <int R, int LPGT, bool DEFER, bool KEYS, bool SSD = false, bool LDSMIN = false, bool OUT8 = false>
 __global__ __launch_bounds__(64, 2) void k_match_ring(MatchParams a) {
     using P = PackCfg<COST_SAD4, R>;
+    static_assert(!OUT8 || (!KEYS && !SSD), "the u8 plane holds the SAD ring's disparity output only");
     constexpr int NW = P::NW, NC = P::NC, W2 = 2 * R + 1;
     static_assert(!LDSMIN || (LPGT == 32 && R <= 5), "the LDS fold is laid out for two 32-lane groups of 32-bit keys");
     constexpr bool PK = R >= 6;
@@ -26,7 +27,8 @@
     if (bz) {
         a.L += bz * a.fs_in;
         a.R += bz * a.fs_in;
-        a.out += bz * a.fs_out;
+        if constexpr (OUT8) a.out8 += bz * a.fs_out;
+        else a.out += bz * a.fs_out;
         if constexpr (KEYS) a.keys += bz * a.fs_out;
     }
     const int lane = threadIdx.x;
@@ -54,11 +56,16 @@
     build_ring_packs<R, 3, RG_DPL>(a, yc, cL0, NL, cR0, NRlog, c0, Lw, Rw, lane);
 
     if (!KEYS && bx == 0 && !a.margins_done) {
-        const int16_t inv = (int16_t)((a.minD - 1) * 16);
+        using OT = typename std::conditional<OUT8, uint8_t, int16_t>::type;
+        const OT inv = OUT8 ? (OT)0 : (OT)((a.minD - 1) * 16);
+        OT* const obase = [&] {
+            if constexpr (OUT8) return a.out8;
+            else return a.out;
+        }();
 #pragma unroll
         for (int q = 0; q < 4; ++q) {
             if (y + q >= a.row1) break;
-            int16_t* orow = a.out + (size_t)(y + q) * a.opitch;
+            OT* orow = obase + (size_t)(y + q) * a.opitch;
             for (int x = lane; x < a.X0; x += 64) orow[x] = inv;
             for (int x = a.X1 + lane; x < a.W; x += 64) orow[x] = inv;
         }
@@ -76,8 +83,8 @@
 #pragma unroll
     for (int k = 0; k < RG_DPL; ++k) {
         const int idx = 4 * l + k;
-        const uint32_t base = PK ? 0u : idx < a.D ? (uint32_t)idx : (SSD ? a.pad_key : 0x8000u << 16) | (uint32_t)idx;
-        lab[k] = (uint32_t)idx;
+        lab[k] = (uint32_t)idx + (OUT8 ? 1u : 0u);
+        const uint32_t base = PK ? 0u : idx < a.D ? lab[k] : (SSD ? a.pad_key : 0x8000u << 16) | lab[k];
 #pragma unroll
         for (int q = 0; q < RQ; ++q) h[k][q] = base;
     }
@@ -105,10 +112,11 @@
     const int eq = LDSMIN ? lane >> 4 : jq;
     const int exs = LDSMIN ? xw + ((lane >> 2) & 1) * S : xs;
     const int eb = (LDSMIN ? ((lane >> 3) & 1) + 2 * (lane & 1) : ju + pofs) - 2 * R;
-    constexpr int OB = KEYS ? 4 : 2;
+    constexpr int OB = KEYS ? 4 : OUT8 ? 1 : 2;
     const int ooff = OB * ((y + eq) * a.opitch + exs + eb);
-    const auto orsrc = KEYS ? __builtin_amdgcn_make_buffer_rsrc(a.keys, 0, 0x7FFFFFFF, 0x00020000)
-                            : __builtin_amdgcn_make_buffer_rsrc(a.out, 0, 0x7FFFFFFF, 0x00020000);
+    const auto orsrc = KEYS   ? __builtin_amdgcn_make_buffer_rsrc(a.keys, 0, 0x7FFFFFFF, 0x00020000)
+                       : OUT8 ? __builtin_amdgcn_make_buffer_rsrc(a.out8, 0, 0x7FFFFFFF, 0x00020000)
+                              : __builtin_amdgcn_make_buffer_rsrc(a.out, 0, 0x7FFFFFFF, 0x00020000);
     const int emax = (LDSMIN ? (lane & 2) == 0 && y + eq < a.row1
                              : (l & 1) == 0 && l < (join2 ? 32 : 16) && y + jq < a.row1)
                          ? max(0, min(S, a.X1 - exs)) : 0;
@@ -116,6 +124,7 @@
     auto emit_key = [&](uint32_t key, int tt) {
         const int off = (unsigned)(tt + eb) < (unsigned)emax ? ooff + OB * tt : (int)0x80000000u;
         if constexpr (KEYS) __builtin_amdgcn_raw_buffer_store_b32(key, orsrc, off, 0, 0);
+        else if constexpr (OUT8) __builtin_amdgcn_raw_buffer_store_b8((uint8_t)key, orsrc, off, 0, 0);
         else __builtin_amdgcn_raw_buffer_store_b16(
             (uint16_t)key_disp16(key, SSD ? (1u << a.dbits) - 1u : 0xFFFFu, a.minD), orsrc, off, 0, 0);
     };
@@ -370,15 +379,21 @@
     return best;
 }
 
-template <int R, int LPG, bool KEYS, bool SSD>
+bool ring_defer() {
+    static const bool defer = env_flag("SV_RING_DEFER", true);
+    return defer;
+}
+
+template <int R, int LPG, bool KEYS, bool SSD, bool OUT8>
 int launch_ring_rl(const MatchParams& a, size_t lds, bool ldsmin, hipStream_t s) {
-    static const bool defer = env_flag("SV_RING_DEFER", true);
+    const bool defer = ring_defer();
     void (*fn)(MatchParams);
     if constexpr (SSD) fn = k_match_ring<R, LPG, R != 5, false, true>;
     else if constexpr (KEYS) fn = k_match_ring<R, LPG, R != 5, true>;
+    else if constexpr (OUT8) fn = k_match_ring<R, LPG, R != 5, false, false, false, true>;
     else fn = (defer && R != 5) ? k_match_ring<R, LPG, R != 5, false> : k_match_ring<R, LPG, false, false>;
     if constexpr (R == 4 && LPG == 32 && !KEYS && !SSD) {
-        if (ldsmin) fn = k_match_ring<R, LPG, false, false, false, true>;
+        if (ldsmin) fn = k_match_ring<R, LPG, false, false, false, true, OUT8>;
     }
     if (lds > 65536) {
         hipError_t e = hipFuncSetAttribute((const void*)fn, hipFuncAttributeMaxDynamicSharedMemorySize, (int)lds);
@@ -399,17 +414,17 @@
     hipLaunchKernelGGL(fn, grid, dim3(64), lds, s, b);
     return (int)hipGetLastError();
 }
-template <int R, bool KEYS, bool SSD = false>
+template <int R, bool KEYS, bool SSD = false, bool OUT8 = false>
 int launch_ring_r(const MatchParams& a, size_t lds, bool ldsmin, hipStream_t s) {
     switch (a.lpg) {
-        case 16: return launch_ring_rl<R, 16, KEYS, SSD>(a, lds, ldsmin, s);
-        case 32: return launch_ring_rl<R, 32, KEYS, SSD>(a, lds, ldsmin, s);
-        case 64: return launch_ring_rl<R, 64, KEYS, SSD>(a, lds, ldsmin, s);
+        case 16: return launch_ring_rl<R, 16, KEYS, SSD, OUT8>(a, lds, ldsmin, s);
+        case 32: return launch_ring_rl<R, 32, KEYS, SSD, OUT8>(a, lds, ldsmin, s);
+        case 64: return launch_ring_rl<R, 64, KEYS, SSD, OUT8>(a, lds, ldsmin, s);
     }
     return (int)hipErrorInvalidValue;
 }
 
-template <bool KEYS, bool SSD = false>
+template <bool KEYS, bool SSD = false, bool OUT8 = false>
 int launch_ring(const MatchParams& a0, hipStream_t s) {
     MatchParams a = a0;
     a.lpg = ring_lpg(a.D);
@@ -429,12 +444,12 @@
         return (int)hipErrorInvalidValue;
     } else {
         switch (a.r) {
-            case 2: return launch_ring_r<2, KEYS>(a, lds, ldsmin, s);
-            case 3: return launch_ring_r<3, KEYS>(a, lds, ldsmin, s);
-            case 4: return launch_ring_r<4, KEYS>(a, lds, ldsmin, s);
-            case 5: return launch_ring_r<5, KEYS>(a, lds, ldsmin, s);
-            case 6: return launch_ring_r<6, KEYS>(a, lds, ldsmin, s);
-            case 7: return launch_ring_r<7, KEYS>(a, lds, ldsmin, s);
+            case 2: return launch_ring_r<2, KEYS, false, OUT8>(a, lds, ldsmin, s);
+            case 3: return launch_ring_r<3, KEYS, false, OUT8>(a, lds, ldsmin, s);
+            case 4: return launch_ring_r<4, KEYS, false, OUT8>(a, lds, ldsmin, s);
+            case 5: return launch_ring_r<5, KEYS, false, OUT8>(a, lds, ldsmin, s);
+            case 6: return launch_ring_r<6, KEYS, false, OUT8>(a, lds, ldsmin, s);
+            case 7: return launch_ring_r<7, KEYS, false, OUT8>(a, lds, ldsmin, s);
         }
         return (int)hipErrorInvalidValue;
     }
@@ -481,7 +496,17 @@
     return ((long long)(nf > 1 ? nf - 1 : 0) * fs_out + (long long)(row1 + 3) * opitch + 64 + 3) & ~3LL;
 }
 
+bool ring_out8(int cost, int win, int num_disp, int row1, int opitch, int W) {
+    const bool fits = (long long)(row1 + 3) * opitch + W + 64 < 0x7FFFFFFFLL;
+    return cost == COST_SAD && num_disp >= 1 && num_disp <= 255 && ring_kind(cost, win, num_disp) && fits &&
+           ring_defer();
+}
+
 int launch_match_ring(const MatchParams& a, int cost, hipStream_t s) {
+    if (a.out8) {
+        if (!ring_out8(cost, a.win, a.D, a.row1, a.opitch, a.W)) return (int)hipErrorInvalidValue;
+        return launch_ring<false, false, true>(a, s);
+    }
     const bool ring_fits = 2LL * ((long long)(a.row1 + 3) * a.opitch + a.W + 64) < 0x7FFFFFFFLL;
     if (ring_kind(cost, a.win, a.D) && ring_fits) return launch_ring<false>(a, s);
     if (ring_ssd(cost, a.win, a.D) && ring_fits) return launch_ring<false, true>(a, s);
diff --git a/stereovision_amd/csrc/sv_median.hip b/stereovision_amd/csrc/sv_median.hip
--- a/stereovision_amd/csrc/sv_median.hip
+++ b/stereovision_amd/csrc/sv_median.hip
@@ -140,11 +140,13 @@
     }
 }
 
-template <int HF, bool WH>
-__global__ __launch_bounds__(256) void k_median_i16(const int16_t* __restrict__ in, int H, int W,
+template <int HF, bool WH, typename TI = int16_t>
+__global__ __launch_bounds__(256) void k_median_i16(const TI* __restrict__ in, int H, int W,
                                                     int row0, int row1, float* __restrict__ disp,
                                                     PostParams pp, long long fs_in, long long fs_out,
                                                     HarrisParams hp) {
+    constexpr bool IN8 = sizeof(TI) == 1;
+    static_assert(!IN8 || WH, "the u8 plane is the fused call's own map: unchecked lookups only");
     if (HF != 0 && (int)blockIdx.x >= hp.mbx) {
         const int w = (int)(blockIdx.x - hp.mbx) * 4 + (int)(threadIdx.x >> 6);
         const int y0 = row0 + (int)blockIdx.y * MQ_H;
@@ -161,8 +163,10 @@
         }
         return;
     }
-    constexpr int TC = MQ_W + 4, TR = MQ_H + 2;
-    __shared__ uint32_t t2[TR][TC];
+    constexpr int CO = IN8 ? 2 : 0;
+    constexpr int TC = MQ_W + 4 + 2 * CO, TR = MQ_H + 2;
+    static_assert(!IN8 || TC % 4 == 0, "the dword fill stores aligned 16-byte groups");
+    __shared__ __attribute__((aligned(16))) uint32_t t2[TR][TC];
     __shared__ __attribute__((aligned(8))) uint32_t srt[MQ_H / 4][4][TC];
     if (blockIdx.z) {
         in += blockIdx.z * fs_in;
@@ -176,7 +180,36 @@
         if (pp.out_d8) pp.out_d8 += o;
     }
     const int x0 = blockIdx.x * MQ_W, y0 = row0 + blockIdx.y * MQ_H;
-    {
+    bool dwfill = false;
+    if constexpr (IN8)
+        dwfill = x0 >= 4 && x0 + MQ_W + 3 <= W - 1 && y0 >= 2 && y0 + TR - 1 <= H - 1 && (W & 3) == 0 &&
+                 ((uintptr_t)in & 3) == 0;
+    if (dwfill) {
+        if constexpr (IN8) {
+            const uint32_t two = 2u * (uint32_t)W;
+            auto fill4 = [&](int r, int j, uint32_t off) {
+                const char* p = reinterpret_cast<const char*>(in);
+                const uint32_t a = *reinterpret_cast<const uint32_t*>(p + off);
+                const uint32_t b = *reinterpret_cast<const uint32_t*>(p + (uint32_t)(off + two));
+                uint4 v;
+                v.x = __builtin_amdgcn_perm(b, a, 0x0c040c00u);
+                v.y = __builtin_amdgcn_perm(b, a, 0x0c050c01u);
+                v.z = __builtin_amdgcn_perm(b, a, 0x0c060c02u);
+                v.w = __builtin_amdgcn_perm(b, a, 0x0c070c03u);
+                *reinterpret_cast<uint4*>(&t2[r][4 * j]) = v;
+            };
+            const int j = (int)(threadIdx.x & 31), rr = (int)(threadIdx.x >> 5);
+            const uint32_t off = (uint32_t)(y0 - 2 + rr) * W + (uint32_t)(x0 - 4 + 4 * j);
+            fill4(rr, j, off);
+            fill4(rr + 8, j, off + 8u * (uint32_t)W);
+            if (threadIdx.x < 64) fill4(rr + 16, j, off + 16u * (uint32_t)W);
+            const int e = (int)threadIdx.x - 64;
+            if ((unsigned)e < 2u * TR) {
+                const int r = e >> 1, je = 32 + (e & 1);
+                fill4(r, je, (uint32_t)(y0 - 2 + r) * W + (uint32_t)(x0 - 4 + 4 * je));
+            }
+        }
+    } else {
         const int c = (int)(threadIdx.x & (MQ_W - 1)), g = (int)(threadIdx.x / MQ_W);
         constexpr int G = 256 / MQ_W;
         static_assert(TR % G == 0, "row groups must tile the pair rows");
@@ -188,7 +221,7 @@
             for (int k = 0; k < TR / G; ++k) {
                 const uint16_t a = (uint16_t)at(in, off);
                 const uint16_t b = (uint16_t)at(in, off + two);
-                t2[g + G * k][c] = (uint32_t)a | ((uint32_t)b << 16);
+                t2[g + G * k][c + CO] = (uint32_t)a | ((uint32_t)b << 16);
                 off += step;
             }
         } else {
@@ -197,7 +230,7 @@
                 const int r = g + G * k;
                 const uint16_t a = (uint16_t)at(in, (uint32_t)clampi(y0 - 2 + r, 0, H - 1) * W + cx);
                 const uint16_t b = (uint16_t)at(in, (uint32_t)clampi(y0 + r, 0, H - 1) * W + cx);
-                t2[r][c] = (uint32_t)a | ((uint32_t)b << 16);
+                t2[r][c + CO] = (uint32_t)a | ((uint32_t)b << 16);
             }
         }
         if (threadIdx.x < 4 * TR) {
@@ -205,11 +238,12 @@
             const uint32_t cxe = (uint32_t)clampi(x0 - 2 + ce, 0, W - 1);
             const uint16_t a = (uint16_t)at(in, (uint32_t)clampi(y0 - 2 + r, 0, H - 1) * W + cxe);
             const uint16_t b = (uint16_t)at(in, (uint32_t)clampi(y0 + r, 0, H - 1) * W + cxe);
-            t2[r][ce] = (uint32_t)a | ((uint32_t)b << 16);
+            t2[r][ce + CO] = (uint32_t)a | ((uint32_t)b << 16);
         }
     }
     __syncthreads();
     const int tx = 2 * (int)(threadIdx.x & 63), tb = 4 * (int)(threadIdx.x >> 6);
+    const int tc = tx + CO;
     {
         auto sort_col = [&](int g4, int c) {
             s2 w[4];
@@ -219,18 +253,18 @@
 #pragma unroll
             for (int i = 0; i < 4; ++i) srt[g4 >> 2][i][c] = __builtin_bit_cast(uint32_t, w[i]);
         };
-        sort_col(tb, tx);
-        sort_col(tb, tx + 1);
-        if (threadIdx.x < 16) sort_col(4 * (threadIdx.x >> 2), MQ_W + (threadIdx.x & 3));
+        sort_col(tb, tc);
+        sort_col(tb, tc + 1);
+        if (threadIdx.x < 16) sort_col(4 * (threadIdx.x >> 2), MQ_W + CO + (threadIdx.x & 3));
     }
     __syncthreads();
 
     s2 cm[16], own[2][4];
 #pragma unroll
     for (int i = 0; i < 4; ++i) {
-        const uint2 p0 = *reinterpret_cast<const uint2*>(&srt[tb >> 2][i][tx]);
-        const uint2 p1 = *reinterpret_cast<const uint2*>(&srt[tb >> 2][i][tx + 2]);
-        const uint2 p2 = *reinterpret_cast<const uint2*>(&srt[tb >> 2][i][tx + 4]);
+        const uint2 p0 = *reinterpret_cast<const uint2*>(&srt[tb >> 2][i][tc]);
+        const uint2 p1 = *reinterpret_cast<const uint2*>(&srt[tb >> 2][i][tc + 2]);
+        const uint2 p2 = *reinterpret_cast<const uint2*>(&srt[tb >> 2][i][tc + 4]);
         own[0][i] = as_s2(p0.x);
         cm[0 * 4 + i] = as_s2(p0.y);
         cm[1 * 4 + i] = as_s2(p1.x);
@@ -256,9 +290,9 @@
     for (int h = 0; h < 2; ++h) {
         s2 q[6];
         {
-            const uint2 p0 = *reinterpret_cast<const uint2*>(&t2[tb + 5 * h][tx]);
-            const uint2 p1 = *reinterpret_cast<const uint2*>(&t2[tb + 5 * h][tx + 2]);
-            const uint2 p2 = *reinterpret_cast<const uint2*>(&t2[tb + 5 * h][tx + 4]);
+            const uint2 p0 = *reinterpret_cast<const uint2*>(&t2[tb + 5 * h][tc]);
+            const uint2 p1 = *reinterpret_cast<const uint2*>(&t2[tb + 5 * h][tc + 2]);
+            const uint2 p2 = *reinterpret_cast<const uint2*>(&t2[tb + 5 * h][tc + 4]);
             q[0] = as_s2(p0.x); q[1] = as_s2(p0.y); q[2] = as_s2(p1.x);
             q[3] = as_s2(p1.y); q[4] = as_s2(p2.x); q[5] = as_s2(p2.y);
         }
@@ -291,7 +325,18 @@
     med[tb + 2][tx >> 1] = mp[2];
     med[tb + 3][tx >> 1] = mp[3];
     __syncthreads();
-    auto post = [&](int mv) { return WH ? post_median_whole(pp, mv) : post_median(pp, mv); };
+    [[maybe_unused]] const int vb = pp.lut_m0 >> 4;
+    [[maybe_unused]] const float fvb = (float)vb;
+    auto post = [&](int mv) {
+        if constexpr (IN8) return lut_entry(pp, (uint32_t)mv);
+        else return WH ? post_median_whole(pp, mv) : post_median(pp, mv);
+    };
+    auto dispf = [&](int mv) {
+        if constexpr (IN8) return (float)(uint32_t)mv + fvb;
+        else return (float)mv / 16.0f;
+    };
+    auto m16 = [&](int mv) { return (int16_t)(IN8 ? (mv + vb) * 16 : mv); };
+    auto d8 = [&](int mv) { return (uint8_t)((IN8 ? mv + vb : mv >> 4) - pp.d8_base); };
     const bool vec = (W & 3) == 0 &&
                      (((uintptr_t)disp | (uintptr_t)pp.out_a | (uintptr_t)pp.out_b) & 15) == 0 &&
                      (((uintptr_t)pp.out_u8 | (uintptr_t)pp.out_bgr | (uintptr_t)pp.out_d8) & 3) == 0 &&
@@ -302,19 +347,24 @@
         const int y = y0 + r, x = x0 + c4;
         if (y >= row1 || x >= W) continue;
         const uint2 raw = *reinterpret_cast<const uint2*>(&med[r][c4 >> 1]);
-        const int mv[4] = {(int)(int16_t)(raw.x & 0xFFFF), (int)(int16_t)(raw.x >> 16),
-                           (int)(int16_t)(raw.y & 0xFFFF), (int)(int16_t)(raw.y >> 16)};
+        const int mv[4] = {IN8 ? (int)(raw.x & 0xFFFF) : (int)(int16_t)(raw.x & 0xFFFF),
+                           IN8 ? (int)(raw.x >> 16) : (int)(int16_t)(raw.x >> 16),
+                           IN8 ? (int)(raw.y & 0xFFFF) : (int)(int16_t)(raw.y & 0xFFFF),
+                           IN8 ? (int)(raw.y >> 16) : (int)(int16_t)(raw.y >> 16)};
         const uint32_t i = (uint32_t)y * W + x;
         if (vec) {
             if (disp)
                 at(reinterpret_cast<float4*>(disp), i >> 2) =
-                    make_float4((float)mv[0] / 16.0f, (float)mv[1] / 16.0f, (float)mv[2] / 16.0f, (float)mv[3] / 16.0f);
-            if (pp.out_m16) at(reinterpret_cast<uint2*>(pp.out_m16), i >> 2) = raw;
+                    make_float4(dispf(mv[0]), dispf(mv[1]), dispf(mv[2]), dispf(mv[3]));
+            if (pp.out_m16)
+                at(reinterpret_cast<uint2*>(pp.out_m16), i >> 2) =
+                    !IN8 ? raw
+                         : make_uint2((uint32_t)(uint16_t)m16(mv[0]) | ((uint32_t)(uint16_t)m16(mv[1]) << 16),
+                                      (uint32_t)(uint16_t)m16(mv[2]) | ((uint32_t)(uint16_t)m16(mv[3]) << 16));
             if (pp.out_d8)
                 at(reinterpret_cast<uint32_t*>(pp.out_d8), i >> 2) =
-                    (uint32_t)(uint8_t)((mv[0] >> 4) - pp.d8_base) | ((uint32_t)(uint8_t)((mv[1] >> 4) - pp.d8_base) << 8) |
-                    ((uint32_t)(uint8_t)((mv[2] >> 4) - pp.d8_base) << 16) |
-                    ((uint32_t)(uint8_t)((mv[3] >> 4) - pp.d8_base) << 24);
+                    (uint32_t)d8(mv[0]) | ((uint32_t)d8(mv[1]) << 8) | ((uint32_t)d8(mv[2]) << 16) |
+                    ((uint32_t)d8(mv[3]) << 24);
             if (pp.mode == POST_NONE) continue;
             PostVals o[4];
 #pragma unroll
@@ -337,9 +387,9 @@
 #pragma unroll
         for (int q = 0; q < 4; ++q) {
             if (x + q >= W) break;
-            if (disp) at(disp, i + q) = (float)mv[q] / 16.0f;
-            if (pp.out_m16) at(pp.out_m16, i + q) = (int16_t)mv[q];
-            if (pp.out_d8) at(pp.out_d8, i + q) = (uint8_t)((mv[q] >> 4) - pp.d8_base);
+            if (disp) at(disp, i + q) = dispf(mv[q]);
+            if (pp.out_m16) at(pp.out_m16, i + q) = m16(mv[q]);
+            if (pp.out_d8) at(pp.out_d8, i + q) = d8(mv[q]);
             if (pp.mode == POST_NONE) continue;
             const PostVals o = post(mv[q]);
             store_post(pp, i + q, o);
@@ -389,9 +439,11 @@
 
 }
 
-int launch_median_i16(const int16_t* in, int H, int W, int row0, int row1, float* disp,
-                      const PostParams& pp, hipStream_t s, int nf, long long fs_in, long long fs_out,
-                      const HarrisParams* harris) {
+namespace {
+template <typename TI>
+int launch_median_t(const TI* in, int H, int W, int row0, int row1, float* disp, const PostParams& pp,
+                    hipStream_t s, int nf, long long fs_in, long long fs_out, const HarrisParams* harris) {
+    constexpr bool IN8 = sizeof(TI) == 1;
     if (row1 <= row0 || nf <= 0) return 0;
     if ((long long)H * W >= (1LL << 30)) return (int)hipErrorInvalidValue;
     HarrisParams hp{};
@@ -405,12 +457,35 @@
     hp.mbx = (W + MQ_W - 1) / MQ_W;
     const bool wh = pp.lut_unchecked && pp.mode != POST_NONE && pp.lut_shift == 4 && pp.lut_n > 0 &&
                     pp.lut_cap >= kLutWholeSpan;
-    void (*fn)(const int16_t*, int, int, int, int, float*, PostParams, long long, long long, HarrisParams) =
-        wh ? (hbx == 0 ? k_median_i16<0, true> : hp.form ? k_median_i16<2, true> : k_median_i16<1, true>)
-           : (hbx == 0 ? k_median_i16<0, false> : hp.form ? k_median_i16<2, false> : k_median_i16<1, false>);
+    void (*fn)(const TI*, int, int, int, int, float*, PostParams, long long, long long, HarrisParams);
+    if constexpr (IN8) {
+        if (!wh || !median_u8_ok(pp)) return (int)hipErrorInvalidValue;
+        fn = hbx == 0 ? k_median_i16<0, true, uint8_t> : hp.form ? k_median_i16<2, true, uint8_t>
+                                                                 : k_median_i16<1, true, uint8_t>;
+    } else {
+        fn = wh ? (hbx == 0 ? k_median_i16<0, true> : hp.form ? k_median_i16<2, true> : k_median_i16<1, true>)
+                : (hbx == 0 ? k_median_i16<0, false> : hp.form ? k_median_i16<2, false> : k_median_i16<1, false>);
+    }
     hipLaunchKernelGGL(fn, dim3(hp.mbx + hbx, (row1 - row0 + MQ_H - 1) / MQ_H, nf),
                        dim3(256), 0, s, in, H, W, row0, row1, disp, pp, fs_in, fs_out, hp);
     return (int)hipGetLastError();
+}
+}
+
+int launch_median_i16(const int16_t* in, int H, int W, int row0, int row1, float* disp,
+                      const PostParams& pp, hipStream_t s, int nf, long long fs_in, long long fs_out,
+                      const HarrisParams* harris) {
+    return launch_median_t(in, H, W, row0, row1, disp, pp, s, nf, fs_in, fs_out, harris);
+}
+
+bool median_u8_ok(const PostParams& pp) {
+    return pp.lut_unchecked && pp.mode != POST_NONE && pp.lut_shift == 4 && pp.num_disp >= 1 && pp.num_disp <= 255 &&
+           pp.lut_n == pp.num_disp + 1 && pp.lut_m0 == (pp.min_disp - 1) * 16 && pp.lut_cap >= kLutWholeSpan;
+}
+
+int launch_median_u8(const uint8_t* in, int H, int W, int row0, int row1, float* disp, const PostParams& pp,
+                     hipStream_t s, int nf, long long fs_in, long long fs_out, const HarrisParams* harris) {
+    return launch_median_t(in, H, W, row0, row1, disp, pp, s, nf, fs_in, fs_out, harris);
 }
 
 int launch_post_m16(const int16_t* in, long long n, float* disp, const PostParams& pp, hipStream_t s) {
```

After: 32770, median of 6. About the same (+0.9%).
